# AtomGradient/swift-qwen3-tts

Measured on AMD Instinct MI355X. Metric: codec_tokens_per_s, higher is better.
Workload: dtype bf16

## Files before the change

### include/q3tts.h

```cpp
#ifndef Q3TTS_H
#define Q3TTS_H

#include <stddef.h>
#include <stdint.h>

#ifdef __cplusplus
extern "C" {
#endif

#define Q3TTS_ABI_VERSION 4

typedef struct q3tts_model q3tts_model;

typedef enum {
    Q3TTS_OK = 0,
    Q3TTS_ERR_MODEL_NOT_INITIALIZED = 1,
    Q3TTS_ERR_GENERATION_FAILED = 2,
    Q3TTS_ERR_INVALID_INPUT = 3,
    Q3TTS_ERR_AUDIO_DECODING_FAILED = 4,
    Q3TTS_ERR_AUDIO_ENCODING_FAILED = 5,
    Q3TTS_ERR_IO = 6,
    Q3TTS_ERR_DEVICE = 7,
    Q3TTS_ERR_CANCELLED = 8,
    Q3TTS_ERR_BUSY = 9
} q3tts_status;

typedef struct {
    int32_t device;
    int32_t max_batch;
    int32_t max_frames;
    int32_t max_prompt;
    int32_t use_graph;
    int32_t weights_from_broadcast;
    int32_t n_streams;
    int32_t codec_overlap_cus;
    int32_t codec_fp32;
    int32_t output_sample_rate;
    float speed;
    int32_t request_speeds;
} q3tts_load_opts;

void q3tts_default_load_opts(q3tts_load_opts* o);

typedef struct {
    q3tts_load_opts base;
    float pitch;
} q3tts_load_opts_ex;

void q3tts_default_load_opts_ex(q3tts_load_opts_ex* o);

q3tts_status q3tts_model_load(const char* model_dir, const q3tts_load_opts* opts, q3tts_model** out);
q3tts_status q3tts_model_load_ex(const char* model_dir, const q3tts_load_opts_ex* opts, q3tts_model** out);
void q3tts_model_free(q3tts_model* m);

const char* q3tts_last_error(const q3tts_model* m);

q3tts_status q3tts_model_arena(q3tts_model* m, void** device_ptr, size_t* bytes);

typedef struct {
    char tts_model_type[32];
    int32_t sample_rate;
    int32_t supports_voice_cloning;
    int32_t has_voice_cloning;
    int32_t hidden_size, num_layers, vocab_size, text_vocab_size, num_code_groups;
    int32_t cp_hidden_size, cp_num_layers, cp_vocab_size;
    int32_t codec_eos_token_id;
    int32_t samples_per_frame;
    int32_t max_batch;
    int64_t weight_bytes;
    int32_t speaker_embedding_dim;
    int32_t max_samples_per_frame;
} q3tts_model_info;
q3tts_status q3tts_model_get_info(const q3tts_model* m, q3tts_model_info* out);

typedef struct { char bytes[128]; } q3tts_comm_id;
q3tts_status q3tts_comm_get_unique_id(q3tts_comm_id* out);
q3tts_status q3tts_model_broadcast(q3tts_model* m, const q3tts_comm_id* id, int32_t rank, int32_t world, int32_t root);
q3tts_status q3tts_model_arena_checksum(q3tts_model* m, uint64_t* out);

int32_t q3tts_model_num_speakers(const q3tts_model* m);
const char* q3tts_model_speaker_name(const q3tts_model* m, int32_t i);

typedef struct {
    const int32_t* text_ids;
    int32_t n_text_ids;
    const int32_t* instruct_ids;
    int32_t n_instruct_ids;
    int32_t target_token_count;
    const char* speaker;
    const char* language;
    int32_t max_tokens;
    float speed;
    const float* ref_audio;
    int64_t n_ref_samples;
    const int32_t* ref_text_ids;
    int32_t n_ref_text_ids;
    int32_t route;
} q3tts_request;

#define Q3TTS_ROW_TEMPERATURE        1u
#define Q3TTS_ROW_TOP_K              2u
#define Q3TTS_ROW_TOP_P              4u
#define Q3TTS_ROW_REPETITION_PENALTY 8u
#define Q3TTS_ROW_SEED               16u
typedef struct {
    uint32_t set;
    float temperature;
    int32_t top_k;
    float top_p;
    float repetition_penalty;
    uint64_t seed;
} q3tts_row_sampling;

typedef struct {
    float temperature;
    int32_t top_k;
    float top_p;
    float repetition_penalty;
    uint64_t seed;
    int32_t force_frames;
    int32_t audio_chunk_frames;
    int32_t audio_window_frames;
    int32_t audio_lookahead_frames;
    uint32_t row_base;
    const q3tts_row_sampling* per_request;
    int32_t audio_stream_reference;
} q3tts_sampling;
void q3tts_default_sampling(q3tts_sampling* s);

typedef struct {
    int32_t prompt_token_count;
    int32_t generation_token_count;
    double prefill_time;
    double generate_time;
    double tokens_per_second;
    double peak_memory_usage;
} q3tts_gen_info;

typedef enum {
    Q3TTS_EVENT_TOKEN = 0, Q3TTS_EVENT_INFO = 1, Q3TTS_EVENT_AUDIO = 2,
    Q3TTS_EVENT_AUDIO_CHUNK = 3
} q3tts_event_kind;
typedef struct {
    q3tts_event_kind kind;
    int32_t request_index;
    int32_t token;
    const q3tts_gen_info* info;
    const float* pcm;
    int64_t n_samples;
    int64_t sample_offset;
} q3tts_event;
typedef void (*q3tts_event_cb)(void* user, const q3tts_event* ev);

typedef struct {
    q3tts_status status;
    float* pcm;
    int64_t n_samples;
    int32_t* codes;
    int32_t n_frames;
    q3tts_gen_info info;
} q3tts_result;

q3tts_status q3tts_generate(q3tts_model* m, const q3tts_request* reqs, int32_t n_reqs,
                            const q3tts_sampling* sampling, q3tts_event_cb cb, void* user,
                            q3tts_result* results);
void q3tts_result_free(q3tts_result* results, int32_t n);

typedef struct q3tts_job q3tts_job;
q3tts_status q3tts_generate_begin(q3tts_model* m, const q3tts_request* reqs, int32_t n_reqs,
                                  const q3tts_sampling* sampling, q3tts_event_cb cb, void* user, int32_t more_follows,
                                  q3tts_job** job);
q3tts_status q3tts_generate_end(q3tts_model* m, q3tts_job* job, q3tts_result* results);

q3tts_status q3tts_generate_queued(q3tts_model* m, const q3tts_request* reqs, int32_t n_reqs, int32_t slots,
                                   const q3tts_sampling* sampling, q3tts_event_cb cb, void* user, q3tts_result* results);

typedef struct q3tts_voice q3tts_voice;
q3tts_status q3tts_voice_create(q3tts_model* m, const float* ref_audio, int64_t n_ref_samples, const int32_t* ref_text_ids,
                                int32_t n_ref_text_ids, q3tts_voice** out);
q3tts_status q3tts_voice_create_rate(q3tts_model* m, const float* ref_audio, int64_t n_ref_samples, int32_t sample_rate,
                                     const int32_t* ref_text_ids, int32_t n_ref_text_ids, q3tts_voice** out);
void q3tts_voice_free(q3tts_model* m, q3tts_voice* v);
typedef struct {
    int32_t ref_frames, ref_text_tokens;
    int64_t n_ref_samples, device_bytes;
} q3tts_voice_info;
q3tts_status q3tts_voice_get_info(const q3tts_voice* v, q3tts_voice_info* out);
q3tts_status q3tts_generate_voices(q3tts_model* m, const q3tts_request* reqs, const q3tts_voice* const* voices, int32_t n_reqs,
                                   const q3tts_sampling* sampling, q3tts_event_cb cb, void* user, q3tts_result* results);
q3tts_status q3tts_generate_queued_voices(q3tts_model* m, const q3tts_request* reqs, const q3tts_voice* const* voices,
                                          int32_t n_reqs, int32_t slots, const q3tts_sampling* sampling, q3tts_event_cb cb,
                                          void* user, q3tts_result* results);

typedef struct q3tts_session q3tts_session;
typedef struct {
    int32_t slots;
    int32_t max_pending;
    int32_t max_ref_frames;
} q3tts_session_opts;
typedef struct {
    int64_t submitted, pending, running, completed, cancelled;
    int64_t frame_steps, admissions;
} q3tts_session_stats;
q3tts_status q3tts_session_open(q3tts_model* m, const q3tts_session_opts* opts, const q3tts_sampling* sampling, q3tts_event_cb cb,
                                void* user, q3tts_session** out);
q3tts_status q3tts_session_submit(q3tts_session* s, const q3tts_request* req, const q3tts_voice* voice ,
                                  const q3tts_row_sampling* rs , int64_t* ticket);
q3tts_status q3tts_session_cancel(q3tts_session* s, int64_t ticket);
q3tts_status q3tts_session_wait(q3tts_session* s, int64_t ticket, int32_t timeout_ms , q3tts_result* out,
                                int32_t* ready);
q3tts_status q3tts_session_get_stats(const q3tts_session* s, q3tts_session_stats* out);
q3tts_status q3tts_session_close(q3tts_session* s, int32_t drain);

typedef struct {
    int64_t open, starved, appended_tokens, starve_events;
} q3tts_session_text_stats;
q3tts_status q3tts_session_submit_open(q3tts_session* s, const q3tts_request* req, const q3tts_row_sampling* rs ,
                                       int64_t* ticket);
q3tts_status q3tts_session_append_text(q3tts_session* s, int64_t ticket, const int32_t* ids, int32_t n, int32_t final);
q3tts_status q3tts_session_get_text_stats(const q3tts_session* s, q3tts_session_text_stats* out);

q3tts_status q3tts_resample(q3tts_model* m, const float* in, int64_t n_in, int32_t in_rate, int32_t out_rate, int32_t centred,
                            float* out, int64_t cap, int64_t* n_out);

q3tts_status q3tts_model_get_speed(const q3tts_model* m, float* effective_speed, int32_t* hs, int32_t* delay_samples);
q3tts_status q3tts_time_stretch(q3tts_model* m, const float* in, int64_t n_in, float speed, int32_t causal, float* out, int64_t cap,
                                int64_t* n_out);

q3tts_status q3tts_model_get_pitch(const q3tts_model* m, float* effective_semitones, int32_t* hp, int32_t* ho, int32_t* delay_samples);
q3tts_status q3tts_pitch_shift(q3tts_model* m, const float* in, int64_t n_in, float semitones, float* out, int64_t cap, int64_t* n_out);

q3tts_status q3tts_request_speed_info(const q3tts_model* m, float speed, float* effective_speed, int32_t* hs, int32_t* delay_samples,
                                      int32_t* samples_per_frame);

q3tts_status q3tts_codec_decode(q3tts_model* m, const int32_t* codes, const int32_t* n_frames,
                                int32_t batch, int32_t max_frames, float* pcm, int64_t* audio_lengths);

q3tts_status q3tts_codec_decode_streamed(q3tts_model* m, const int32_t* codes, const int32_t* n_frames, int32_t batch,
                                         int32_t max_frames, int32_t chunk_frames, int32_t window, int32_t lookahead, float* pcm);

q3tts_status q3tts_codec_decode_streamed_prefixed(q3tts_model* m, const int32_t* codes, const int32_t* n_prefix, const int32_t* n_frames,
                                                  int32_t batch, int32_t max_frames, int32_t chunk_frames, int32_t window,
                                                  int32_t lookahead, float* pcm);

q3tts_status q3tts_codec_encode(q3tts_model* m, const float* audio, int64_t n_samples, int32_t* codes,
                                int32_t cap_frames, int32_t* n_frames);
int32_t q3tts_codec_encoded_frames(const q3tts_model* m, int64_t n_samples);

q3tts_status q3tts_speaker_embedding(q3tts_model* m, const float* audio, int64_t n_samples, int32_t sample_rate,
                                     float* out, int32_t cap);

void q3tts_pcm_to_int16(const float* pcm, int64_t n_samples, int16_t* out);
q3tts_status q3tts_write_wav(const char* path, const float* pcm, int64_t n_samples, int32_t sample_rate);

typedef struct q3tts_tokenizer q3tts_tokenizer;
q3tts_status q3tts_tokenizer_load(const char* path, q3tts_tokenizer** out);
void q3tts_tokenizer_free(q3tts_tokenizer* t);
q3tts_status q3tts_tokenizer_encode(const q3tts_tokenizer* t, const char* utf8, int32_t* ids, int32_t cap, int32_t* n);

typedef struct {
    double prefill_ms;
    double decode_ms;
    double codec_ms;
    int32_t frame_steps;
    int32_t rows;
    int64_t kv_bytes_read;
    double frontend_ms;
    double first_audio_ms;
    int32_t launches_per_frame_step;
} q3tts_timing;
q3tts_status q3tts_last_timing(const q3tts_model* m, q3tts_timing* out);


q3tts_status q3tts_debug_prepare_inputs(q3tts_model* m, const q3tts_request* req,
                                        uint16_t* input_embeds, int32_t cap_prompt, int32_t* n_prompt,
                                        uint16_t* trailing, int32_t cap_trailing, int32_t* n_trailing,
                                        uint16_t* tts_pad);

q3tts_status q3tts_debug_generate_forced(q3tts_model* m, const q3tts_request* reqs, int32_t n_reqs,
                                         const q3tts_sampling* sampling, const int32_t* forced_codes,
                                         int32_t n_frames, uint16_t* talker_logits, uint16_t* cp_logits,
                                         int32_t* sampled);

q3tts_status q3tts_debug_sample(q3tts_model* m, const uint16_t* logits, int32_t rows, int32_t V,
                                const q3tts_sampling* sampling, const uint8_t* seen,
                                int32_t suppress_lo, int32_t suppress_hi, int32_t eos_id,
                                uint32_t row0, uint32_t draw, int32_t* tokens);

q3tts_status q3tts_debug_text_resume(q3tts_model* m, int32_t H, int32_t V, const uint16_t* tables, const int32_t* codes,
                                     const uint16_t* text_row, uint16_t* out_h, float* out_ss, int32_t* out_state);

q3tts_status q3tts_debug_linear(q3tts_model* m, const uint16_t* x, const uint16_t* W, const uint16_t* bias,
                                int32_t M, int32_t K, int32_t N, uint16_t* y);

typedef struct {
    int32_t n_heads, n_kv, B;
    float eps, scale;
    int32_t max_pages;
    int32_t fixed_len;
    int32_t identity_pages;
    int32_t chunk;
    int32_t chunk_r_base;
    int32_t nt_kv;
    int32_t n_pos;
    int32_t n_pages;
    const uint16_t* qkv;
    const uint16_t* qn_w;
    const uint16_t* kn_w;
    const uint16_t* rope_cos;
    const uint16_t* rope_sin;
    const int32_t* kv_len;
    const uint8_t* active;
    const int32_t* block_table;
    const int32_t* chunk_n_prompt;
    uint16_t* kpool;
    uint16_t* vpool;
    uint16_t* out;
} q3tts_attn_debug;
q3tts_status q3tts_debug_attention(q3tts_model* m, const q3tts_attn_debug* a);

typedef struct {
    int32_t mode, geometry_only;
    int32_t M, K, N;
    int32_t xMB, yMB, ss_ld, y_cols;
    int32_t epi, act_silu, resid, nt_weights, y_tiled;
    int32_t norm, quant, has_bias;
    int32_t ss_count, norm_dim;
    float norm_eps;
    int32_t rider_M, rider_H, rider_MB, rider_ss_count;
    float rider_eps;
    int32_t rode;
    int32_t tall;
    int32_t tall_shape;
    int32_t split, mbw, nw, ch, np, gx, ntw;
    int32_t tm;
    const uint16_t* x;
    const void* W;
    const uint16_t* scales;
    const uint16_t* biases;
    const void* W_up;
    const uint16_t* scales_up;
    const uint16_t* biases_up;
    const uint16_t* bias;
    const uint16_t* norm_w;
    const float* ss_in;
    const uint16_t* rider_h;
    const uint16_t* rider_w;
    const float* rider_ss_in;
    uint16_t* y;
    float* ss_out;
    uint16_t* rider_out;
    float* rider_ss_out;
} q3tts_gemm_debug;
q3tts_status q3tts_debug_gemm(q3tts_model* m, q3tts_gemm_debug* a);

typedef struct {
    int32_t kind, geometry_only, split;
    int32_t B, Tmax, ppf, hist, margin;
    int32_t Cin, N, K, dil;
    int32_t ldx, ldo, ldr, ldx2;
    int32_t act, pre_act, shift, reflect, post_C;
    int32_t x_f32, res_is_out;
    int32_t family;
    int32_t BN;
    int32_t pro, pw_depth, KT, X32, CT2, PT, wdb;
    int32_t grid_x, grid_y, grid_z;
    int64_t lds_bytes;
    const int32_t* frames;
    const void* x;
    const float* x2;
    const float* w;
    const float* w2;
    const float* bias;
    const float* bias2;
    const float* scale;
    const float* snake_alpha;
    const float* snake_beta;
    const float* act2_alpha;
    const float* act2_beta;
    const float* post_alpha;
    const float* post_beta;
    const void* res;
    void* out;
    void* out2;
    float* pcm;
    int32_t* nonfinite;
} q3tts_conv_debug;
q3tts_status q3tts_debug_conv(q3tts_model* m, q3tts_conv_debug* a);

typedef struct {
    int32_t op, check_only;
    int32_t p[16];
    float f[4];
    const void* in[8];
    int64_t in_bytes[8];
    void* io[4];
    int64_t io_bytes[4];
} q3tts_rowop_debug;
q3tts_status q3tts_debug_rowop(q3tts_model* m, q3tts_rowop_debug* a);

typedef struct {
    float temperature;
    int32_t top_k;
    float top_p;
    float rep_penalty;
    uint64_t seed;
    uint32_t row0;
    int32_t mask_eos;
} q3tts_lm_sampling_params;
typedef struct {
    int32_t slot, n_trailing, max_frames;
    uint32_t row_key;
    int32_t text_open;
    int32_t pad_;
    q3tts_lm_sampling_params sp;
} q3tts_lm_admit_desc;
typedef struct {
    int32_t slot, src_row, n_new, close, max_frames, pad_;
} q3tts_lm_text_desc;
typedef struct {
    int32_t op, check_only;
    int32_t p[32];
    const void* in[14];
    int64_t in_bytes[14];
    void* io[18];
    int64_t io_bytes[18];
} q3tts_lmop_debug;
q3tts_status q3tts_debug_lmop(q3tts_model* m, q3tts_lmop_debug* a);

q3tts_status q3tts_debug_codec_stage(q3tts_model* m, const int32_t* codes, int32_t n_frames,
                                     const char* stage, float* out, int64_t cap_floats, int32_t* T, int32_t* C);

q3tts_status q3tts_debug_prefix_states(q3tts_model* m, int32_t* n_states, int64_t* device_bytes, int64_t* n_restored);

q3tts_status q3tts_debug_stretch_rows(q3tts_model* m, const float* x, const int32_t* lens, const int32_t* hops, int32_t B,
                                      int64_t x_stride, float* y, int64_t y_stride);

q3tts_status q3tts_debug_resample_ratio(q3tts_model* m, const float* x, const int32_t* lens, int32_t B, int64_t row_stride, int64_t in_units,
                                        int64_t out_units, int32_t centred, int32_t clamp, int32_t hist, float* y, int64_t y_stride);

q3tts_status q3tts_debug_codec_stream_slots(q3tts_model* m, const int32_t* codes, const int32_t* n_frames, int32_t n_reqs,
                                            int32_t max_frames, int32_t slots, int32_t burst, int32_t chunk_frames, int32_t window,
                                            int32_t lookahead, float* pcm);

q3tts_status q3tts_debug_build_decode_codes(q3tts_model* m, const int32_t* refs, const int32_t* ref_T, const int32_t* gen,
                                            const int32_t* n_frames, int32_t R, int32_t gen_stride, int32_t Fdec, int32_t misalign,
                                            int32_t* out);

void q3tts_debug_set_codec_scratch(uint64_t bytes);

void q3tts_debug_reload_env(void);

q3tts_status q3tts_debug_frontend_stage(q3tts_model* m, const float* audio, int64_t n_samples, const char* stage,
                                        float* out, int64_t cap_floats, int32_t* T, int32_t* C);

#ifdef __cplusplus
}
#endif
#endif
```

### swift-qwen3-tts_amd/csrc/debug_env.cc

```cpp
#include <atomic>
#include <cstdlib>
#include <mutex>

#include "kernels.h"

namespace q3 {

namespace {
std::mutex g_mu;
std::atomic<const DebugEnv*> g_env{nullptr};

bool flag(const char* name) { return std::getenv(name) != nullptr; }
int number(const char* name, int dflt) {
    const char* e = std::getenv(name);
    return e && *e ? std::atoi(e) : dflt;
}

const DebugEnv* read_env() {
    DebugEnv* d = new DebugEnv{};
    d->gemm_no_row_split = flag("Q3TTS_GEMM_NO_ROW_SPLIT");
    d->gemm_one_pair = flag("Q3TTS_GEMM_ONE_PAIR");
    d->gemm_parent_forms = number("Q3TTS_GEMM_PARENT_FORMS", 0) != 0;
    d->no_tall_gemm = flag("Q3TTS_NO_TALL_GEMM");
    d->tall_shape = number("Q3TTS_TALL_SHAPE", 0);
    d->chunk_qsplit = number("Q3TTS_CHUNK_QSPLIT", 0);
    d->conv_no_pw = flag("Q3TTS_CONV_NO_PW");
    d->nt_off = std::getenv("Q3TTS_NT") && number("Q3TTS_NT", 1) == 0;
    d->serial_jobs = number("Q3TTS_SERIAL_JOBS", 0) != 0;
    d->fail_back_half = number("Q3TTS_TEST_FAIL_BACK_HALF", 0) != 0;
    d->no_prefix_cache = number("Q3TTS_NO_PREFIX_CACHE", 0) != 0;
    return d;
}
}

const DebugEnv& debug_env() {
    const DebugEnv* e = g_env.load(std::memory_order_acquire);
    if (!e) {
        std::lock_guard<std::mutex> lk(g_mu);
        e = g_env.load(std::memory_order_acquire);
        if (!e) {
            e = read_env();
            g_env.store(e, std::memory_order_release);
        }
    }
    return *e;
}

void debug_env_reload() {
    std::lock_guard<std::mutex> lk(g_mu);
    g_env.store(read_env(), std::memory_order_release);
}

}
```

### swift-qwen3-tts_amd/csrc/engine_debug.cc

```cpp
#include "engine_stream.h"

#include "frontend.h"

namespace q3 {

void Engine::debug_frontend_stage(const float* audio, int64_t n_samples, const char* stage, float* out, int64_t cap, int* T, int* C) {
    Q3_CHECK(fe_ != nullptr, 1, "Model not initialized: Speech tokenizer encoder not available");
    Q3_CHECK(audio && n_samples > 0 && stage, 3, "Invalid input: empty audio or stage name");
    const float* a = upload_audio(audio, n_samples);
    StageCapture cap_s;
    cap_s.name = stage;
    static const char* kSpeaker[] = {"mel", "h0", "h1", "h2", "h3", "mfa", "pooled"};
    bool is_spk = false;
    for (const char* s : kSpeaker) is_spk = is_spk || cap_s.name == s;
    if (is_spk) {
        Q3_CHECK(m_->has_speaker_encoder, 1, "Model not initialized: Speaker encoder not available for this model");
        spk_f32_.grow(size_t(m_->cfg.talker.hidden_size));
        fe_->speaker_embedding(a, n_samples, spk_f32_, &cap_s);
    } else {
        Q3_CHECK(m_->has_codec_encoder, 1, "Model not initialized: Speech tokenizer encoder not available");
        const int Tq = fe_->encoded_frames(n_samples);
        ref_codes_dev_.grow(size_t(16) * Tq);
        fe_->encode(a, n_samples, ref_codes_dev_, &cap_s);
    }
    Q3_HIP(hipStreamSynchronize(st_));
    Q3_CHECK(!cap_s.data.empty(), 3, std::string("Invalid input: unknown front-end stage '") + stage + "'");
    Q3_CHECK(int64_t(cap_s.data.size()) <= cap, 3, "Invalid input: output buffer too small");
    std::memcpy(out, cap_s.data.data(), cap_s.data.size() * 4);
    *T = cap_s.T;
    *C = cap_s.C;
}

void Engine::debug_prepare_inputs(const q3tts_request& req, uint16_t* input_embeds, int cap_prompt, int* n_prompt,
                                  uint16_t* trailing, int cap_trailing, int* n_trailing, uint16_t* tts_pad) {
    q3tts_sampling sp{};
    q3tts_default_sampling(&sp);
    std::vector<ResolvedRequest> rr{resolve(req, sp)};
    if (rr[0].clone) prepare_clone_rows(rr);
    std::vector<int> np, nt;
    assemble_prompts(rr, np, nt);
    const int H = m_->cfg.talker.hidden_size;
    Q3_CHECK(np[0] <= cap_prompt && nt[0] <= cap_trailing, 3, "Invalid input: output buffers too small");
    Q3_HIP(hipStreamSynchronize(st_));
    Q3_HIP(hipMemcpy(input_embeds, prompt_, size_t(np[0]) * H * 2, hipMemcpyDeviceToHost));
    Q3_HIP(hipMemcpy(trailing, trailing_, size_t(nt[0]) * H * 2, hipMemcpyDeviceToHost));
    Q3_HIP(hipMemcpy(tts_pad, tts_pad_, size_t(H) * 2, hipMemcpyDeviceToHost));
    *n_prompt = np[0];
    *n_trailing = nt[0];
}

void Engine::debug_sample(const uint16_t* logits, int rows, int V, const q3tts_sampling& sp, const uint8_t* seen,
                          int suppress_lo, int suppress_hi, int eos_id, uint32_t row0, uint32_t draw, int32_t* tokens) {
    Q3_CHECK(rows >= 1 && rows <= Bm_ && V <= m_->cfg.talker.vocab_size, 3, "debug_sample: rows/V out of range");
    Q3_CHECK(draw % 16 == 0, 3, "debug_sample: draw must be a multiple of 16 (frame * 16)");
    const int Vt = m_->cfg.talker.vocab_size;
    Q3_HIP(hipMemcpy2D(tk_.logits, size_t(Vt) * 2, logits, size_t(V) * 2, size_t(V) * 2, size_t(rows), hipMemcpyHostToDevice));
    if (seen) Q3_HIP(hipMemcpy(seen_, seen, size_t(rows) * V, hipMemcpyHostToDevice));
    std::vector<int32_t> fr((size_t)(rows), int32_t(draw / 16)), big((size_t)(rows), 1 << 30);
    Q3_HIP(hipMemcpy(n_frames_, fr.data(), size_t(rows) * 4, hipMemcpyHostToDevice));
    Q3_HIP(hipMemcpy(max_frames_, big.data(), size_t(rows) * 4, hipMemcpyHostToDevice));
    Q3_HIP(hipMemset(finished_, 0, size_t(rows)));
    Q3_HIP(hipMemset(active_, 1, size_t(rows)));
    std::vector<SamplingParams> sph;
    for (int r = 0; r < rows; ++r) sph.push_back(fold_sampling(sp, r, row0));
    Q3_HIP(hipMemcpy(sp_dev_, sph.data(), sph.size() * sizeof(SamplingParams), hipMemcpyHostToDevice));
    SamplerArgs sa{};
    sa.logits = tk_.logits; sa.ldl = Vt; sa.V = V; sa.sp = sp_dev_;
    sa.is_talker = (eos_id >= 0 || suppress_hi > suppress_lo || seen) ? 1 : 0;
    sa.suppress_lo = suppress_lo; sa.suppress_hi = suppress_hi; sa.eos_id = eos_id;
    sa.seen = seen ? seen_ : nullptr; sa.cb = 0; sa.n_frames = n_frames_; sa.max_frames = max_frames_;
    sa.finished = finished_; sa.active = active_; sa.kv_len = kv_len_; sa.advance = 0;
    sa.cur_codes = cur_codes_; sa.codes = codes_; sa.Fmax = 0; sa.B = rows; sa.H = m_->cfg.talker.hidden_size;
    launch_sampler(sa, st_);
    Q3_HIP(hipStreamSynchronize(st_));
    std::vector<int32_t> cc((size_t)(rows) * 16);
    Q3_HIP(hipMemcpy(cc.data(), cur_codes_, cc.size() * 4, hipMemcpyDeviceToHost));
    for (int r = 0; r < rows; ++r) tokens[r] = cc[size_t(r) * 16];
    Q3_HIP(hipMemset(seen_, 0, size_t(rows) * V));
}

void Engine::debug_linear(const uint16_t* x, const uint16_t* W, const uint16_t* bias, int M, int K, int N, uint16_t* y) {
    Q3_CHECK(M >= 1 && M <= 1024 && K % 8 == 0 && N >= 1, 3, "debug_linear: unsupported shape");
    const int Kp = int(align_up(size_t(K), 128)), Np = int(align_up(size_t(N), 16)), Mp = int(align_up(size_t(M), 16));
    uint16_t *dW = nullptr, *dWt = nullptr, *dx = nullptr, *dy = nullptr, *db = nullptr;
    Q3_HIP(hipMalloc(reinterpret_cast<void**>(&dW), size_t(N) * K * 2));
    Q3_HIP(hipMalloc(reinterpret_cast<void**>(&dWt), size_t(Np) * Kp * 2));
    Q3_HIP(hipMalloc(reinterpret_cast<void**>(&dx), size_t(Mp) * Kp * 2));
    Q3_HIP(hipMalloc(reinterpret_cast<void**>(&dy), size_t(Mp) * Np * 2));
    Q3_HIP(hipMalloc(reinterpret_cast<void**>(&db), size_t(Np) * 2));
    Q3_HIP(hipMemset(dWt, 0, size_t(Np) * Kp * 2));
    Q3_HIP(hipMemset(dx, 0, size_t(Mp) * Kp * 2));
    Q3_HIP(hipMemset(db, 0, size_t(Np) * 2));
    Q3_HIP(hipMemcpy(dW, W, size_t(N) * K * 2, hipMemcpyHostToDevice));
    uint16_t* dxl = nullptr;
    Q3_HIP(hipMalloc(reinterpret_cast<void**>(&dxl), size_t(Mp) * Kp * 2));
    Q3_HIP(hipMemset(dxl, 0, size_t(Mp) * Kp * 2));
    Q3_HIP(hipMemcpy2D(dxl, size_t(Kp) * 2, x, size_t(K) * 2, size_t(K) * 2, size_t(M), hipMemcpyHostToDevice));
    launch_tile_rows(dxl, Kp, dx, Mp / 16, Mp, Kp, st_);
    if (bias) Q3_HIP(hipMemcpy(db, bias, size_t(N) * 2, hipMemcpyHostToDevice));
    launch_tile_weights(dW, N, K, dWt, Kp / 128, 0, 1, st_);
    LinearW L;
    L.w = dWt; L.bias = bias ? db : nullptr; L.N = N; L.K = K; L.Np = Np; L.Kp = Kp;
    GemmArgs ga{};
    ga.W = dWt; ga.x = dx; ga.xMB = Mp / 16; ga.M = M; ga.Mpad = Mp; ga.N = Np; ga.K = Kp; ga.epi = 0; ga.y = dy; ga.ldy = Np;
    ga.bias = L.bias; ga.ss_ld = Mp;
    launch_gemm_skinny(ga, st_);
    Q3_HIP(hipStreamSynchronize(st_));
    Q3_HIP(hipMemcpy2D(y, size_t(N) * 2, dy, size_t(Np) * 2, size_t(N) * 2, size_t(M), hipMemcpyDeviceToHost));
    for (void* p : {(void*)dW, (void*)dWt, (void*)dx, (void*)dxl, (void*)dy, (void*)db})
        if (p) (void)hipFree(p);
}

void Engine::debug_text_resume(int H, int V, const uint16_t* tables, const int32_t* codes, const uint16_t* text, uint16_t* out_h,
                               float* out_ss, int32_t* out_state) {
    Q3_CHECK(H >= 128 && H <= 4096 && H % 128 == 0 && V >= 1 && V <= 4096, 3, "debug_text_resume: H must be a multiple of 128 up to 4096, V up to 4096");
    Q3_CHECK(tables && codes && text && out_h && out_ss && out_state, 3, "Invalid input: null argument");
    for (int g = 0; g < 16; ++g) Q3_CHECK(codes[g] >= 0 && codes[g] < V, 3, "debug_text_resume: code outside the tables");
    constexpr int B = 2, row = 1, Tmax = 2;
    DevBuf<uint16_t> d_tab, d_trailing, d_pad, d_h, d_hl, d_text;
    DevBuf<const uint16_t*> d_cp;
    DevBuf<int32_t> d_i32;
    DevBuf<uint8_t> d_u8;
    DevBuf<float> d_ss;
    DevBuf<TextAppendDesc> d_desc;
    d_tab.grow(size_t(16) * V * H);
    d_trailing.grow(size_t(B) * Tmax * H);
    d_pad.grow(size_t(H));
    d_h.grow(size_t(16) * H);
    d_hl.grow(size_t(16) * H);
    d_text.grow(size_t(H));
    d_cp.grow(15);
    d_i32.grow(32 + 10);
    d_u8.grow(8);
    d_ss.grow(B);
    d_desc.grow(1);
    Q3_HIP(hipMemcpy(d_tab, tables, size_t(16) * V * H * 2, hipMemcpyHostToDevice));
    Q3_HIP(hipMemcpy(d_text, text, size_t(H) * 2, hipMemcpyHostToDevice));
    Q3_HIP(hipMemset(d_pad, 0, size_t(H) * 2));
    std::vector<const uint16_t*> cp(15);
    for (int g = 1; g < 16; ++g) cp[size_t(g - 1)] = d_tab + size_t(g) * V * H;
    Q3_HIP(hipMemcpy(d_cp, cp.data(), 15 * sizeof(const uint16_t*), hipMemcpyHostToDevice));
    int32_t* cur = d_i32;
    int32_t *n_tr = cur + 32, *t_idx = n_tr + 2, *n_fr = t_idx + 2, *max_fr = n_fr + 2, *cp_len = max_fr + 2;
    uint8_t *fin = d_u8, *act = fin + 2, *topen = act + 2, *starved = topen + 2;
    FrameEndArgs fe{};
    fe.cur_codes = cur; fe.codec_emb = d_tab; fe.cp_emb = d_cp;
    fe.trailing = d_trailing; fe.n_trailing = n_tr; fe.trailing_idx = t_idx; fe.Tmax = Tmax;
    fe.tts_pad = d_pad; fe.h = d_h; fe.hMB = 1; fe.ss_out = d_ss; fe.H = H; fe.B = B; fe.groups = 16;
    fe.n_frames = n_fr; fe.max_frames = max_fr; fe.finished = fin; fe.active = act; fe.cp_len = cp_len;
    fe.text_open = topen; fe.starved = starved;
    auto reset = [&](int n_trailing, int open) {
        std::vector<int32_t> hi(42, 0);
        for (int g = 0; g < 16; ++g) hi[size_t(16 + g)] = codes[g];
        hi[32 + row] = n_trailing;
        hi[38] = hi[39] = 100;
        hi[40] = hi[41] = 15;
        const uint8_t hu[8] = {1, 0, 0, 1, 0, uint8_t(open), 0, 0};
        const float hs[2] = {-1.f, -1.f};
        Q3_HIP(hipMemcpy(d_i32, hi.data(), hi.size() * 4, hipMemcpyHostToDevice));
        Q3_HIP(hipMemcpy(d_u8, hu, 8, hipMemcpyHostToDevice));
        Q3_HIP(hipMemcpy(d_ss, hs, 8, hipMemcpyHostToDevice));
        Q3_HIP(hipMemset(d_h, 0xEE, size_t(16) * H * 2));
        Q3_HIP(hipMemset(d_trailing, 0, size_t(B) * Tmax * H * 2));
    };
    auto read = [&](int k) {
        launch_untile_rows(d_h, 1, d_hl, H, 16, H, st_);
        Q3_HIP(hipStreamSynchronize(st_));
        Q3_HIP(hipMemcpy(out_h + size_t(k) * H, d_hl + size_t(row) * H, size_t(H) * 2, hipMemcpyDeviceToHost));
        float hs[2];
        int32_t hi[42];
        uint8_t hu[8];
        Q3_HIP(hipMemcpy(hs, d_ss, 8, hipMemcpyDeviceToHost));
        Q3_HIP(hipMemcpy(hi, d_i32, sizeof(hi), hipMemcpyDeviceToHost));
        Q3_HIP(hipMemcpy(hu, d_u8, 8, hipMemcpyDeviceToHost));
        out_ss[k] = hs[row];
        int32_t* o = out_state + size_t(k) * 8;
        o[0] = hi[36 + row]; o[1] = hi[34 + row]; o[2] = hi[32 + row]; o[3] = hu[row]; o[4] = hu[2 + row]; o[5] = hu[4 + row];
        o[6] = hu[6 + row]; o[7] = hi[40 + row];
    };
    reset(1, 0);
    Q3_HIP(hipMemcpy(d_trailing + size_t(row) * Tmax * H, d_text, size_t(H) * 2, hipMemcpyDeviceToDevice));
    launch_frame_end(fe, st_);
    read(0);
    reset(0, 1);
    launch_frame_end(fe, st_);
    read(1);
    TextAppendDesc d{};
    d.slot = row; d.src_row = 0; d.n_new = 1;
    Q3_HIP(hipMemcpy(d_desc, &d, sizeof(d), hipMemcpyHostToDevice));
    TextAppendArgs ta{};
    ta.desc = d_desc; ta.src = d_text; ta.eos_row = d_pad; ta.trailing = d_trailing; ta.n_trailing = n_tr; ta.text_open = topen;
    ta.max_frames = max_fr; ta.slots = B; ta.fe = fe;
    launch_text_append_rows(ta, &d, 1, st_);
    read(2);
}

void Engine::debug_build_decode_codes(const int32_t* refs, const int32_t* ref_T, const int32_t* gen, const int32_t* n_frames, int R,
                                      int gen_stride, int Fdec, bool misalign, int32_t* out) {
    size_t ref_total = 0;
    for (int r = 0; r < R; ++r) {
        Q3_CHECK(ref_T[r] >= 0 && n_frames[r] >= 0 && n_frames[r] <= gen_stride, 3, "Invalid input: frame counts out of range");
        ref_total += size_t(16) * ref_T[r];
    }
    Q3_CHECK(ref_total == 0 || refs, 3, "Invalid input: null argument");
    const size_t off = misalign ? 1 : 0, n_gen = size_t(R) * gen_stride * 16, n_out = size_t(R) * Fdec * 16;
    DevBuf<int32_t> d_ref, d_gen, d_out;
    DevBuf<DecodeRowDesc> d_desc;
    d_ref.grow(std::max<size_t>(ref_total, 1));
    d_gen.grow(n_gen + off);
    d_out.grow(n_out + off);
    d_desc.grow(size_t(R));
    if (ref_total) Q3_HIP(hipMemcpyAsync(d_ref, refs, ref_total * 4, hipMemcpyHostToDevice, st_));
    Q3_HIP(hipMemcpyAsync(d_gen + off, gen, n_gen * 4, hipMemcpyHostToDevice, st_));
    Q3_HIP(hipMemcpyAsync(d_out + off, out, n_out * 4, hipMemcpyHostToDevice, st_));
    std::vector<DecodeRowDesc> desc((size_t)(R));
    size_t at = 0;
    for (int r = 0; r < R; ++r) {
        desc[size_t(r)] = DecodeRowDesc{ref_T[r] > 0 ? d_ref + at : nullptr, d_gen + off + size_t(r) * gen_stride * 16, ref_T[r], n_frames[r], r, 0};
        at += size_t(16) * ref_T[r];
    }
    Q3_HIP(hipMemcpyAsync(d_desc, desc.data(), desc.size() * sizeof(DecodeRowDesc), hipMemcpyHostToDevice, st_));
    launch_build_decode_codes_rows(desc.data(), d_desc, R, d_out + off, R, Fdec, st_);
    Q3_HIP(hipMemcpyAsync(out, d_out + off, n_out * 4, hipMemcpyDeviceToHost, st_));
    Q3_HIP(hipStreamSynchronize(st_));
}

void Engine::debug_attention(const q3tts_attn_debug& d) {
    Q3_CHECK(d.qkv && d.qn_w && d.kn_w && d.rope_cos && d.rope_sin && d.kpool && d.vpool && d.out, 3, "debug_attention: null argument");
    Q3_CHECK(d.n_kv >= 1 && d.n_kv <= 64 && d.n_heads >= d.n_kv && d.n_heads % d.n_kv == 0 && d.n_heads / d.n_kv <= 4, 3,
             "debug_attention: unsupported GQA ratio");
    Q3_CHECK(d.B >= 1 && d.B <= 256, 3, "debug_attention: batch out of range");
    Q3_CHECK(d.chunk >= 0 && d.chunk <= 16, 3, "debug_attention: at most 16 positions per launch");
    Q3_CHECK(d.max_pages >= 1 && d.max_pages <= 64 && d.n_pages >= 1 && d.n_pages <= 4096 && d.n_pos >= 1 && d.n_pos <= 65536, 3,
             "debug_attention: sizes out of range");
    Q3_CHECK(d.fixed_len >= -1, 3, "debug_attention: fixed_len out of range");
    Q3_CHECK(d.fixed_len >= 0 || d.kv_len, 3, "debug_attention: kv_len missing");
    Q3_CHECK(d.identity_pages || d.block_table, 3, "debug_attention: block_table missing");
    Q3_CHECK(!d.identity_pages || d.B <= d.n_pages, 3, "debug_attention: identity_pages needs a page per row");
    const int B = d.B, C = std::max(d.chunk, 1), rows = C * B;
    const int cap = (d.identity_pages ? 1 : d.max_pages) * kPageTokens;
    for (int b = 0; b < B; ++b) {
        const int len0 = d.fixed_len >= 0 ? d.fixed_len : d.kv_len[b];
        int live = 1;
        if (d.chunk > 1 && d.chunk_n_prompt) {
            const int64_t r0 = int64_t(d.chunk_r_base) + d.chunk_n_prompt[b];
            live = r0 < 0 ? int(std::max<int64_t>(0, C + r0)) : C;
        } else if (d.chunk > 1) {
            live = C;
        }
        Q3_CHECK(len0 >= 0 && len0 <= cap && len0 + live <= cap && len0 + live <= d.n_pos, 3,
                 "debug_attention: cache length beyond the pages or the RoPE tables");
        if (!d.identity_pages)
            for (int pg = 0; pg * kPageTokens < len0 + live; ++pg) {
                const int32_t e = d.block_table[size_t(b) * d.max_pages + pg];
                Q3_CHECK(e >= 0 && e < d.n_pages, 3, "debug_attention: block-table entry outside the pool");
            }
    }
    const int ld = (d.n_heads + 2 * d.n_kv) * kHeadDim, odim = d.n_heads * kHeadDim;
    const int Mp = int(align_up(size_t(rows), 16));
    const size_t pool = size_t(d.n_pages) * d.n_kv * kPageTokens * kHeadDim;
    const size_t tab = size_t(d.n_pos) * kHeadDim;
    DevBuf<uint16_t> qkv, w, rope, kp, vp, ot, ol;
    DevBuf<int32_t> ints;
    DevBuf<uint8_t> act;
    qkv.grow(size_t(rows) * ld);
    w.grow(2 * kHeadDim);
    rope.grow(2 * tab);
    kp.grow(pool);
    vp.grow(pool);
    ot.grow(size_t(Mp) * odim);
    ol.grow(size_t(rows) * odim);
    ints.grow(size_t(B) * (2 + d.max_pages));
    act.grow(size_t(B));
    int32_t *kv_len = ints, *n_prompt = kv_len + B, *bt = n_prompt + B;
    Q3_HIP(hipMemset(ints, 0, size_t(B) * (2 + d.max_pages) * 4));
    Q3_HIP(hipMemcpy(qkv, d.qkv, size_t(rows) * ld * 2, hipMemcpyHostToDevice));
    Q3_HIP(hipMemcpy(w, d.qn_w, kHeadDim * 2, hipMemcpyHostToDevice));
    Q3_HIP(hipMemcpy(w + kHeadDim, d.kn_w, kHeadDim * 2, hipMemcpyHostToDevice));
    Q3_HIP(hipMemcpy(rope, d.rope_cos, tab * 2, hipMemcpyHostToDevice));
    Q3_HIP(hipMemcpy(rope + tab, d.rope_sin, tab * 2, hipMemcpyHostToDevice));
    Q3_HIP(hipMemcpy(kp, d.kpool, pool * 2, hipMemcpyHostToDevice));
    Q3_HIP(hipMemcpy(vp, d.vpool, pool * 2, hipMemcpyHostToDevice));
    if (d.kv_len) Q3_HIP(hipMemcpy(kv_len, d.kv_len, size_t(B) * 4, hipMemcpyHostToDevice));
    if (d.chunk_n_prompt) Q3_HIP(hipMemcpy(n_prompt, d.chunk_n_prompt, size_t(B) * 4, hipMemcpyHostToDevice));
    if (d.block_table) Q3_HIP(hipMemcpy(bt, d.block_table, size_t(B) * d.max_pages * 4, hipMemcpyHostToDevice));
    if (d.active) Q3_HIP(hipMemcpy(act, d.active, size_t(B), hipMemcpyHostToDevice));
    Q3_HIP(hipMemset(ot, 0xff, size_t(Mp) * odim * 2));
    AttnArgs at{};
    at.qkv = qkv; at.ld = ld; at.qn_w = w; at.kn_w = w + kHeadDim; at.eps = d.eps;
    at.rope_cos = rope; at.rope_sin = rope + tab;
    at.kpool = kp; at.vpool = vp;
    at.block_table = bt; at.max_pages = d.max_pages; at.kv_len = kv_len; at.active = d.active ? (const uint8_t*)act : nullptr;
    at.out = ot; at.outMB = Mp / 16; at.n_heads = d.n_heads; at.n_kv = d.n_kv; at.B = B;
    at.scale = d.scale;
    at.fixed_len = d.fixed_len; at.identity_pages = d.identity_pages ? 1 : 0;
    at.chunk = d.chunk; at.chunk_n_prompt = d.chunk_n_prompt ? n_prompt : nullptr; at.chunk_r_base = d.chunk_r_base;
    at.nt_kv = d.nt_kv ? 1 : 0;
    launch_attn_decode(at, st_);
    Q3_HIP(hipGetLastError());
    launch_untile_rows(ot, Mp / 16, ol, odim, rows, odim, st_);
    Q3_HIP(hipStreamSynchronize(st_));
    Q3_HIP(hipMemcpy(d.out, ol, size_t(rows) * odim * 2, hipMemcpyDeviceToHost));
    Q3_HIP(hipMemcpy(d.kpool, kp, pool * 2, hipMemcpyDeviceToHost));
    Q3_HIP(hipMemcpy(d.vpool, vp, pool * 2, hipMemcpyDeviceToHost));
}

void Engine::debug_gemm_check(q3tts_gemm_debug& d, GemmArgs& ga, NormRowsArgs& na) {
    static const uint16_t dummy16 = 0;
    static const uint32_t dummy32 = 0;
    d.rode = d.tall = d.tall_shape = d.split = d.mbw = d.nw = d.ch = d.np = d.gx = d.ntw = d.tm = 0;
    Q3_CHECK(d.mode == 0 || d.mode == 1, 3, "debug_gemm: unknown mode");
    const bool rider = d.mode == 1 || d.rider_M > 0;
    if (rider) {
        Q3_CHECK(d.rider_M >= 1 && d.rider_MB >= 1 && d.rider_MB <= 64 && d.rider_M <= 16 * d.rider_MB, 3, "debug_gemm: rider rows out of range");
        Q3_CHECK(d.rider_H >= 128 && d.rider_H <= 4096 && d.rider_H % 128 == 0, 3, "debug_gemm: rider_H must be a multiple of 128 up to 4096");
        Q3_CHECK(d.geometry_only || (d.rider_h && d.rider_w && d.rider_out), 3, "debug_gemm: null rider argument");
        if (d.rider_ss_in) Q3_CHECK(d.rider_ss_count >= 1 && d.rider_ss_count <= 256, 3, "debug_gemm: at most 256 partial sums of squares per rider row");
        na.hMB = na.outMB = d.rider_MB; na.eps = d.rider_eps; na.M = d.rider_M; na.H = d.rider_H;
        na.ss_count = d.rider_ss_in ? d.rider_ss_count : 0; na.ss_ld = 16 * d.rider_MB;
    }
    if (d.mode == 1) return;
    Q3_CHECK(d.epi == 0 || d.epi == 2 || d.epi == 3, 3, "debug_gemm: unknown epilogue");
    Q3_CHECK(d.M >= 1 && d.M <= 1024, 3, "debug_gemm: M out of range");
    Q3_CHECK(d.K >= 128 && d.K <= 8192 && d.K % 128 == 0, 3, "debug_gemm: K must be a multiple of 128 up to 8192");
    Q3_CHECK(d.N >= 8 && d.N <= 65536 && d.N % (d.epi == 2 ? 8 : 16) == 0, 3, "debug_gemm: N must be a multiple of 16 (epi 2: of 8)");
    const int Mp = int(align_up(size_t(d.M), 16));
    const bool tiled = d.epi != 0 || d.y_tiled;
    Q3_CHECK(d.xMB <= 64 && 16 * d.xMB >= Mp && d.yMB <= 64 && 16 * d.yMB >= Mp && d.ss_ld >= Mp && d.ss_ld <= 4096, 3,
             "debug_gemm: allocation smaller than the padded batch");
    Q3_CHECK(d.y_cols >= d.N && d.y_cols <= d.N + 1024 && d.y_cols % (tiled ? 128 : 8) == 0, 3, "debug_gemm: y_cols");
    Q3_CHECK(d.epi != 2 || (!d.has_bias && !d.act_silu), 3, "debug_gemm: the gate/up epilogue takes no bias or activation");
    Q3_CHECK(d.epi == 0 || !d.act_silu, 3, "debug_gemm: act_silu belongs to epi 0");
    Q3_CHECK(d.epi == 3 || (!d.resid && !d.ss_out), 3, "debug_gemm: resid / ss_out belong to epi 3");
    if (d.norm) Q3_CHECK(d.ss_count >= 1 && d.ss_count <= 4096 && d.norm_dim >= 1, 3, "debug_gemm: norm prologue sizes");
    if (!d.geometry_only) {
        Q3_CHECK(d.x && d.W && d.y, 3, "debug_gemm: null argument");
        Q3_CHECK((d.epi == 2) == (d.W_up != nullptr), 3, "debug_gemm: W_up goes with epi 2");
        Q3_CHECK((d.quant != 0) == (d.scales != nullptr) && (d.quant != 0) == (d.biases != nullptr), 3, "debug_gemm: scales / biases go with quant");
        if (d.epi == 2) Q3_CHECK((d.quant != 0) == (d.scales_up != nullptr) && (d.quant != 0) == (d.biases_up != nullptr), 3, "debug_gemm: scales / biases go with quant");
        Q3_CHECK((d.has_bias != 0) == (d.bias != nullptr), 3, "debug_gemm: bias goes with has_bias");
        Q3_CHECK((d.norm != 0) == (d.norm_w != nullptr) && (d.norm != 0) == (d.ss_in != nullptr), 3, "debug_gemm: norm_w / ss_in go with norm");
    }
    ga.Wsb = d.quant ? &dummy32 : nullptr;
    ga.xMB = d.xMB; ga.M = d.M; ga.Mpad = Mp; ga.N = d.N; ga.K = d.K; ga.epi = d.epi;
    ga.ldy = d.y_cols; ga.y_tiled = d.y_tiled ? 1 : 0; ga.yMB = d.yMB;
    ga.bias = d.has_bias ? &dummy16 : nullptr;
    ga.act_silu = d.act_silu ? 1 : 0;
    ga.norm_w = d.norm ? &dummy16 : nullptr;
    ga.ss_count = d.norm ? d.ss_count : 0; ga.ss_ld = d.ss_ld; ga.norm_dim = d.norm_dim; ga.norm_eps = d.norm_eps;
    ga.nt_weights = d.nt_weights ? 1 : 0; ga.resid = d.resid ? 1 : 0;
    const SkinnyGeom g = skinny_geometry(ga);
    d.tall = g.tall ? 1 : 0;
    if (g.tall) {
        d.tall_shape = gemm_tall_shape(ga);
    } else {
        Q3_CHECK(g.mbw >= 1 && g.mbw <= 4, 3, "debug_gemm: more than 4 row blocks per workgroup");
        d.split = g.split; d.mbw = g.mbw; d.nw = g.nw; d.ch = g.ch; d.np = g.np; d.gx = g.gx; d.ntw = g.ntw ? 1 : 0; d.tm = g.tm ? 1 : 0;
    }
    if (rider) d.rode = gemm_norm_rows_rides(ga, na) ? 1 : 0;
}

namespace {
void host_tile(const uint16_t* src, std::vector<uint16_t>& dst, int rows, int cols) {
    dst.resize(size_t(rows) * cols);
    for (int m = 0; m < rows; ++m)
        for (int k = 0; k < cols; k += 8) std::memcpy(&dst[act_tiled_offset(m, k, rows / 16)], src + size_t(m) * cols + k, 16);
}
void host_untile(const std::vector<uint16_t>& src, uint16_t* dst, int rows, int cols) {
    for (int m = 0; m < rows; ++m)
        for (int k = 0; k < cols; k += 8) std::memcpy(dst + size_t(m) * cols + k, &src[act_tiled_offset(m, k, rows / 16)], 16);
}
}

void Engine::debug_gemm(q3tts_gemm_debug& d) {
    GemmArgs ga{};
    NormRowsArgs na{};
    debug_gemm_check(d, ga, na);
    DevBuf<uint16_t> dx, dy, dbias, dnw, dsrc, dsc, dbi, rh, rw, rout;
    DevBuf<uint8_t> dWt;
    DevBuf<uint32_t> dWq, dsb;
    DevBuf<float> dssi, dsso, rssi, rsso;
    std::vector<uint16_t> tmp;
    auto up16 = [&](DevBuf<uint16_t>& b, const uint16_t* src, size_t n) {
        b.grow(n);
        Q3_HIP(hipMemcpy(b, src, n * 2, hipMemcpyHostToDevice));
    };
    const bool rider = d.mode == 1 || d.rider_M > 0;
    const int rrows = 16 * d.rider_MB;
    if (rider) {
        host_tile(d.rider_h, tmp, rrows, d.rider_H);
        up16(rh, tmp.data(), tmp.size());
        host_tile(d.rider_out, tmp, rrows, d.rider_H);
        up16(rout, tmp.data(), tmp.size());
        up16(rw, d.rider_w, size_t(d.rider_H));
        na.h = rh; na.w = rw; na.out = rout;
        if (d.rider_ss_in) {
            rssi.grow(size_t(d.rider_ss_count) * rrows);
            Q3_HIP(hipMemcpy(rssi, d.rider_ss_in, size_t(d.rider_ss_count) * rrows * 4, hipMemcpyHostToDevice));
            na.ss_in = rssi;
        }
        if (d.rider_ss_out) {
            rsso.grow(size_t(rrows));
            Q3_HIP(hipMemcpy(rsso, d.rider_ss_out, size_t(rrows) * 4, hipMemcpyHostToDevice));
            na.ss_out = rsso;
        }
    }
    const bool tiled = d.mode == 0 && (d.epi != 0 || d.y_tiled);
    const int yrows = 16 * d.yMB, n_tiles = d.mode == 0 ? (d.epi == 2 ? d.N / 8 : d.N / 16) : 0, KC = d.K / 128;
    const size_t n_ss_out = d.mode == 0 ? size_t(d.N / 16) * d.ss_ld : 0;
    if (d.mode == 0) {
        host_tile(d.x, tmp, 16 * d.xMB, d.K);
        up16(dx, tmp.data(), tmp.size());
        if (tiled) {
            host_tile(d.y, tmp, yrows, d.y_cols);
            up16(dy, tmp.data(), tmp.size());
        } else {
            up16(dy, d.y, size_t(yrows) * d.y_cols);
        }
        const size_t wbytes = d.quant ? size_t(n_tiles) * 16 * d.K / 2 : size_t(n_tiles) * 16 * d.K * 2;
        dWt.grow(wbytes);
        Q3_HIP(hipMemset(dWt, 0, wbytes));
        if (d.quant) {
            dsb.grow(size_t(n_tiles) * KC * 64);
            Q3_HIP(hipMemset(dsb, 0, size_t(n_tiles) * KC * 64 * 4));
        }
        const int rpt = d.epi == 2 ? 8 : 16;
        for (int part = 0; part < (d.epi == 2 ? 2 : 1); ++part) {
            const void* W = part ? d.W_up : d.W;
            if (d.quant) {
                dWq.grow(size_t(d.N) * d.K / 8);
                Q3_HIP(hipMemcpy(dWq, W, size_t(d.N) * d.K / 8 * 4, hipMemcpyHostToDevice));
                up16(dsc, part ? d.scales_up : d.scales, size_t(d.N) * d.K / 64);
                up16(dbi, part ? d.biases_up : d.biases, size_t(d.N) * d.K / 64);
                launch_tile_int4(dWq, dsc, dbi, d.N, d.K, dWt, dsb, KC, 0, 1, st_, rpt, 8 * part);
            } else {
                up16(dsrc, static_cast<const uint16_t*>(W), size_t(d.N) * d.K);
                launch_tile_weights(dsrc, d.N, d.K, reinterpret_cast<uint16_t*>(static_cast<uint8_t*>(dWt)), KC, 0, 1, st_, rpt, 8 * part);
            }
            Q3_HIP(hipStreamSynchronize(st_));
        }
        if (d.bias) up16(dbias, d.bias, size_t(d.N));
        if (d.norm) {
            up16(dnw, d.norm_w, size_t(d.K));
            dssi.grow(size_t(d.ss_count) * d.ss_ld);
            Q3_HIP(hipMemcpy(dssi, d.ss_in, size_t(d.ss_count) * d.ss_ld * 4, hipMemcpyHostToDevice));
        }
        if (d.ss_out) {
            dsso.grow(n_ss_out);
            Q3_HIP(hipMemcpy(dsso, d.ss_out, n_ss_out * 4, hipMemcpyHostToDevice));
        }
        ga.W = reinterpret_cast<const uint16_t*>(static_cast<uint8_t*>(dWt));
        ga.Wsb = d.quant ? static_cast<uint32_t*>(dsb) : nullptr;
        ga.x = dx; ga.y = dy;
        ga.bias = d.bias ? static_cast<uint16_t*>(dbias) : nullptr;
        ga.norm_w = d.norm ? static_cast<uint16_t*>(dnw) : nullptr;
        ga.ss_in = d.norm ? static_cast<float*>(dssi) : nullptr;
        ga.ss_out = d.ss_out ? static_cast<float*>(dsso) : nullptr;
    }
    bool launched = true;
    if (d.mode == 1) {
        launch_norm_rows(na, st_);
    } else if (rider) {
        launched = launch_gemm_skinny_with_norm_rows(ga, na, st_);
        Q3_CHECK(launched == (d.rode != 0), 7, "debug_gemm: the rider launch disagrees with gemm_norm_rows_rides");
    } else {
        launch_gemm_skinny(ga, st_);
    }
    Q3_HIP(hipGetLastError());
    Q3_HIP(hipStreamSynchronize(st_));
    if (!launched) return;
    if (d.mode == 0) {
        if (tiled) {
            tmp.resize(size_t(yrows) * d.y_cols);
            Q3_HIP(hipMemcpy(tmp.data(), dy, tmp.size() * 2, hipMemcpyDeviceToHost));
            host_untile(tmp, d.y, yrows, d.y_cols);
        } else {
            Q3_HIP(hipMemcpy(d.y, dy, size_t(yrows) * d.y_cols * 2, hipMemcpyDeviceToHost));
        }
        if (d.ss_out) Q3_HIP(hipMemcpy(d.ss_out, dsso, n_ss_out * 4, hipMemcpyDeviceToHost));
    }
    if (rider) {
        tmp.resize(size_t(rrows) * d.rider_H);
        Q3_HIP(hipMemcpy(tmp.data(), rout, tmp.size() * 2, hipMemcpyDeviceToHost));
        host_untile(tmp, d.rider_out, rrows, d.rider_H);
        if (d.rider_ss_out) Q3_HIP(hipMemcpy(d.rider_ss_out, rsso, size_t(rrows) * 4, hipMemcpyDeviceToHost));
    }
}

static void check_caller_codes(const CodecW& w, const int32_t* codes, const int32_t* n_frames, int batch, int max_frames) {
    for (int b = 0; b < batch; ++b)
        for (int f = 0; f < n_frames[b]; ++f) {
            const int32_t* c = codes + (size_t(b) * max_frames + f) * 16;
            Q3_CHECK(c[0] >= 0 && c[0] < w.cb_first_rows, 3, "Invalid input: first code outside the semantic codebook");
            for (size_t j = 0; j < w.cb_rest.size(); ++j)
                Q3_CHECK(c[1 + j] >= 0 && c[1 + j] < w.cb_rest_rows, 3, "Invalid input: code outside the acoustic codebook");
        }
}

void Engine::codec_decode(const int32_t* codes, const int32_t* n_frames, int batch, int max_frames, float* pcm,
                          int64_t* audio_lengths) {
    Q3_CHECK(m_->has_codec, 1, "Model not initialized: Speech tokenizer not loaded");
    Q3_CHECK(batch >= 1 && max_frames >= 1, 3, "Invalid input: empty codec batch");
    const int up = codec_->upsample();
    std::vector<int> frames((size_t)(batch));
    int Fmax = 0;
    for (int b = 0; b < batch; ++b) {
        Q3_CHECK(n_frames[b] >= 0 && n_frames[b] <= max_frames, 3, "Invalid input: n_frames out of range");
        frames[size_t(b)] = n_frames[b];
        Fmax = std::max(Fmax, n_frames[b]);
    }
    check_caller_codes(m_->codec, codes, n_frames, batch, max_frames);
    DevBuf<int32_t> dcodes;
    dcodes.grow(size_t(batch) * max_frames * 16);
    Q3_HIP(hipMemcpy(dcodes, codes, size_t(batch) * max_frames * 16 * 4, hipMemcpyHostToDevice));
    float* pcm_dev = nullptr;
    hipStream_t cst = codec_stream(false);
    PinnedBuf<int32_t> nf;
    nf.grow(size_t(batch));
    std::memset(nf, 0, size_t(batch) * 4);
    Q3_HIP(hipEventRecord(ev_[2], cst));
    if (Fmax > 0) codec_->decode(dcodes, max_frames, frames, &pcm_dev, std::string(), nullptr, nullptr, nullptr, nf);
    Q3_HIP(hipEventRecord(ev_[3], cst));
    Q3_HIP(hipStreamSynchronize(cst));
    bool bad = false;
    for (int b = 0; b < batch; ++b) bad = bad || nf[b] != 0;
    if (bad && !codec_->fp32_convs()) {
        std::memset(nf, 0, size_t(batch) * 4);
        codec_->decode(dcodes, max_frames, frames, &pcm_dev, std::string(), nullptr, nullptr, nullptr, nf, true);
        Q3_HIP(hipEventRecord(ev_[3], cst));
        Q3_HIP(hipStreamSynchronize(cst));
        bad = false;
        for (int b = 0; b < batch; ++b) bad = bad || nf[b] != 0;
    }
    if (bad) throw Error(4, kCodecRangeMsg);
    float ms = 0;
    Q3_HIP(hipEventElapsedTime(&ms, ev_[2], ev_[3]));
    timing.codec_ms = ms;
    for (int b = 0; b < batch; ++b) {
        const int F = frames[size_t(b)];
        if (F > 0)
            Q3_HIP(hipMemcpy(pcm + size_t(b) * max_frames * up, pcm_dev + size_t(b) * Fmax * up, size_t(F) * up * 4,
                             hipMemcpyDeviceToHost));
        int valid = 0;
        for (int f = 0; f < F; ++f) valid += codes[(size_t(b) * max_frames + f) * 16] > 0 ? 1 : 0;
        audio_lengths[b] = int64_t(valid) * up;
    }
}

void Engine::codec_decode_streamed(const int32_t* codes, const int32_t* n_frames, int batch, int max_frames, int chunk_frames, int window,
                                   int lookahead, float* pcm) {
    Q3_CHECK(m_->has_codec, 1, "Model not initialized: Speech tokenizer not loaded");
    Q3_CHECK(batch >= 1 && max_frames >= 1 && chunk_frames >= 1, 3, "Invalid input: empty codec batch");
    const int up = codec_->upsample();
    DevBuf<int32_t> dcodes;
    PinnedBuf<float> hpcm;
    struct Events {
        std::vector<hipEvent_t> v;
        ~Events() {
            for (auto e : v) (void)hipEventDestroy(e);
        }
    } done;
    dcodes.grow(size_t(batch) * max_frames * 16);
    Q3_HIP(hipMemcpy(dcodes, codes, size_t(batch) * max_frames * 16 * 4, hipMemcpyHostToDevice));
    hpcm.grow(size_t(batch) * max_frames * up);
    std::memset(hpcm, 0, size_t(batch) * max_frames * up * 4);
    std::vector<int> avail((size_t)(batch));
    std::vector<uint8_t> fin((size_t)(batch), 1);
    int Fmax = 0;
    for (int b = 0; b < batch; ++b) {
        Q3_CHECK(n_frames[b] >= 0 && n_frames[b] <= max_frames, 3, "Invalid input: n_frames out of range");
        avail[size_t(b)] = n_frames[b];
        Fmax = std::max(Fmax, n_frames[b]);
    }
    check_caller_codes(m_->codec, codes, n_frames, batch, max_frames);
    hipStream_t cst = codec_stream(false);
    CodecRunner::StreamCfg cfg;
    cfg.rows = batch; cfg.chunk_frames = chunk_frames; cfg.window = window; cfg.lookahead = lookahead; cfg.max_frames = std::max(Fmax, 1);
    codec_->stream_open(cfg);
    try {
        if (window >= 0) {
            std::vector<uint8_t> notyet((size_t)(batch), 0);
            for (int have = chunk_frames; have < Fmax + chunk_frames + lookahead; have += chunk_frames) {
                std::vector<int> a((size_t)(batch));
                for (int b = 0; b < batch; ++b) {
                    a[size_t(b)] = std::min(avail[size_t(b)], have);
                    notyet[size_t(b)] = a[size_t(b)] == avail[size_t(b)] ? 1 : 0;
                }
                codec_->stream_push(dcodes, max_frames, a.data(), notyet.data(), hpcm, size_t(max_frames) * up, done.v);
            }
        }
        codec_->stream_push(dcodes, max_frames, avail.data(), fin.data(), hpcm, size_t(max_frames) * up, done.v);
    } catch (...) {
        codec_->stream_close();
        throw;
    }
    codec_->stream_close();
    Q3_HIP(hipStreamSynchronize(cst));
    for (int b = 0; b < batch; ++b)
        std::memcpy(pcm + size_t(b) * max_frames * up, hpcm + size_t(b) * max_frames * up, size_t(n_frames[b]) * up * 4);
}

void Engine::codec_decode_streamed_prefixed(const int32_t* codes, const int32_t* n_prefix, const int32_t* n_frames, int batch, int max_frames,
                                            int chunk_frames, int window, int lookahead, float* pcm) {
    Q3_CHECK(m_->has_codec, 1, "Model not initialized: Speech tokenizer not loaded");
    Q3_CHECK(batch >= 1 && max_frames >= 1 && chunk_frames >= 1 && window >= 0 && lookahead >= 0, 3, "Invalid input: empty codec batch");
    Q3_CHECK(batch <= Bm_, 3, "Invalid input: batch must be between 1 and max_batch");
    int Fmax = 0, Rmax = 0;
    std::vector<int32_t> total((size_t)(batch));
    for (int b = 0; b < batch; ++b) {
        Q3_CHECK(n_prefix[b] >= 0 && n_frames[b] >= 0 && int64_t(n_prefix[b]) + n_frames[b] <= max_frames, 3,
                 "Invalid input: n_prefix + n_frames out of range");
        total[size_t(b)] = n_prefix[b] + n_frames[b];
        Fmax = std::max(Fmax, n_frames[b]);
        Rmax = std::max(Rmax, n_prefix[b]);
    }
    check_caller_codes(m_->codec, codes, total.data(), batch, max_frames);
    check_stream_chunk(chunk_frames);
    const int up = codec_->upsample();
    DevBuf<int32_t> dcodes;
    dcodes.grow(size_t(batch) * max_frames * 16);
    Q3_HIP(hipMemcpy(dcodes, codes, size_t(batch) * max_frames * 16 * 4, hipMemcpyHostToDevice));
    SlotStream ss(*this, batch, chunk_frames, window, lookahead, std::max(Fmax, 1), false, Rmax);
    ss.hold = false;
    for (int b = 0; b < batch; ++b) ss.admit(b, b, std::max(Fmax, 1), n_prefix[b]);
    std::vector<int> avail((size_t)(batch));
    std::vector<uint8_t> fin((size_t)(batch));
    for (int have = chunk_frames;; have += chunk_frames) {
        bool all = true;
        for (int b = 0; b < batch; ++b) {
            avail[size_t(b)] = std::min(n_frames[b], have);
            fin[size_t(b)] = avail[size_t(b)] == n_frames[b] ? 1 : 0;
            all = all && fin[size_t(b)];
        }
        ss.push(dcodes, max_frames, avail.data(), fin.data());
        if (all) break;
    }
    for (int b = 0; b < batch; ++b) ss.retire(b, n_frames[b]);
    ss.finish();
    for (int b = 0; b < batch; ++b) {
        Q3_CHECK(ss.out[b].complete, 7, "internal error: a row of the prefixed stream was left incomplete");
        std::memcpy(pcm + size_t(b) * Fmax * up, ss.out[b].pcm.get(), size_t(n_frames[b]) * up * 4);
    }
}

void Engine::debug_codec_stream_slots(const int32_t* codes, const int32_t* n_frames, int n_reqs, int max_frames, int slots, int burst,
                                      int chunk_frames, int window, int lookahead, float* pcm) {
    Q3_CHECK(m_->has_codec, 1, "Model not initialized: Speech tokenizer not loaded");
    Q3_CHECK(n_reqs >= 1 && max_frames >= 1 && burst >= 1 && chunk_frames >= 1 && window >= 0 && lookahead >= 0, 3,
             "Invalid input: empty codec batch");
    Q3_CHECK(slots >= 1 && slots <= Bm_, 3, "Invalid input: slots must be between 1 and max_batch");
    for (int i = 0; i < n_reqs; ++i) Q3_CHECK(n_frames[i] >= 0 && n_frames[i] <= max_frames, 3, "Invalid input: n_frames out of range");
    check_caller_codes(m_->codec, codes, n_frames, n_reqs, max_frames);
    check_stream_chunk(chunk_frames);
    const int up = codec_->upsample();
    DevBuf<int32_t> all, scodes;
    all.grow(size_t(n_reqs) * max_frames * 16);
    scodes.grow(size_t(slots) * max_frames * 16);
    Q3_HIP(hipMemcpy(all, codes, size_t(n_reqs) * max_frames * 16 * 4, hipMemcpyHostToDevice));
    SlotStream ss(*this, slots, chunk_frames, window, lookahead, max_frames, false);
    ss.hold = false;
    std::vector<int> copied((size_t)(slots), 0);
    replay_queue_schedule(
        n_frames, n_reqs, slots, burst,
        [&](int s, int r) {
            ss.admit(s, r, max_frames);
            copied[size_t(s)] = 0;
        },
        [&](const int* avail, const uint8_t* fin, const int* req) {
            for (int s = 0; s < slots; ++s) {
                if (req[s] < 0 || avail[s] <= copied[size_t(s)]) continue;
                Q3_HIP(hipMemcpyAsync(scodes + (size_t(s) * max_frames + copied[size_t(s)]) * 16,
                                      all + (size_t(req[s]) * max_frames + copied[size_t(s)]) * 16, size_t(avail[s] - copied[size_t(s)]) * 64,
                                      hipMemcpyDeviceToDevice, ss.cst));
                copied[size_t(s)] = avail[s];
            }
            ss.push(scodes, max_frames, avail, fin);
            for (int s = 0; s < slots; ++s)
                if (req[s] >= 0 && fin[s]) ss.retire(s, avail[s]);
        });
    ss.finish();
    for (int i = 0; i < n_reqs; ++i) {
        Q3_CHECK(ss.out[i].complete, 7, "internal error: a request of the slotted stream was left incomplete");
        std::memcpy(pcm + size_t(i) * max_frames * up, ss.out[i].pcm.get(), size_t(n_frames[i]) * up * 4);
    }
}

void Engine::debug_codec_stage(const int32_t* codes, int n_frames, const char* stage, float* out, int64_t cap, int* T, int* C) {
    Q3_CHECK(m_->has_codec, 1, "Model not initialized: Speech tokenizer not loaded");
    DevBuf<int32_t> dcodes;
    dcodes.grow(size_t(n_frames) * 16);
    Q3_HIP(hipMemcpy(dcodes, codes, size_t(n_frames) * 16 * 4, hipMemcpyHostToDevice));
    std::vector<float> so;
    float* pcm_dev = nullptr;
    (void)codec_stream(false);
    codec_->decode(dcodes, n_frames, {n_frames}, &pcm_dev, stage, &so, T, C);
    Q3_CHECK(int64_t(so.size()) <= cap, 3, "debug_codec_stage: output buffer too small");
    std::memcpy(out, so.data(), so.size() * 4);
}

}
```

### swift-qwen3-tts_amd/csrc/kernels.h

```cpp
#pragma once
#include <hip/hip_runtime.h>

#include <cstdint>

namespace q3 {

struct DebugEnv {
    bool gemm_no_row_split;
    bool gemm_one_pair;
    bool gemm_parent_forms;
    bool no_tall_gemm;
    int tall_shape;
    int chunk_qsplit;
    bool conv_no_pw;
    bool nt_off;
    bool serial_jobs;
    bool fail_back_half;
    bool no_prefix_cache;
};
const DebugEnv& debug_env();
void debug_env_reload();

constexpr int kPageTokens = 64;
constexpr int kHeadDim = 128;

struct NormRowsArgs {
    const uint16_t* h;
    int hMB;
    const uint16_t* w;
    float eps;
    uint16_t* out;
    int outMB;
    float* ss_out;
    int M, H;
    const float* ss_in;
    int ss_count, ss_ld;
};
void launch_norm_rows(const NormRowsArgs& a, hipStream_t st);

struct GemmArgs {
    const uint16_t* W;
    const uint32_t* Wsb;
    const uint16_t* x;
    int xMB;
    int M, Mpad, N, K;
    int epi;
    uint16_t* y;
    int ldy;
    int y_tiled, yMB;
    const uint16_t* bias;
    int act_silu;
    const uint16_t* norm_w;
    const float* ss_in;
    int ss_count, ss_ld, norm_dim;
    float norm_eps;
    int nt_weights;
    int resid;
    float* ss_out;
};
void launch_gemm_skinny(const GemmArgs& a, hipStream_t st);
struct SkinnyGeom {
    bool tall;
    int split, mbw;
    int nw, ch, np;
    int gx;
    bool ntw;
    bool tm;
};
SkinnyGeom skinny_geometry(const GemmArgs& a);
bool launch_gemm_skinny_with_norm_rows(const GemmArgs& a, const NormRowsArgs& n, hipStream_t st);
bool gemm_norm_rows_rides(const GemmArgs& a, const NormRowsArgs& n);
bool launch_gemm_tall(const GemmArgs& a, hipStream_t st);
bool gemm_tall_takes(const GemmArgs& a);
int gemm_tall_shape(const GemmArgs& a);


struct AttnArgs {
    const uint16_t* qkv;
    int ld;
    const uint16_t* qn_w;
    const uint16_t* kn_w;
    float eps;
    const uint16_t* rope_cos;
    const uint16_t* rope_sin;
    uint16_t* kpool;
    uint16_t* vpool;
    const int32_t* block_table;
    int max_pages;
    const int32_t* kv_len;
    const uint8_t* active;
    uint16_t* out;
    int outMB;
    int n_heads, n_kv, B;
    float scale;
    int fixed_len;
    int identity_pages;
    int chunk;
    const int32_t* chunk_n_prompt;
    int chunk_r_base;
    int nt_kv;
};
void launch_attn_decode(const AttnArgs& a, hipStream_t st);

struct FrameEndArgs {
    const int32_t* cur_codes;
    const uint16_t* codec_emb;
    const uint16_t* const* cp_emb;
    const uint16_t* trailing;
    const int32_t* n_trailing;
    int32_t* trailing_idx;
    int Tmax;
    const uint16_t* tts_pad;
    uint16_t* h;
    int hMB, H, B, groups;
    float* ss_out;
    int32_t* n_frames;
    const int32_t* max_frames;
    uint8_t* finished;
    uint8_t* active;
    int32_t* cp_len;
    const uint8_t* text_open;
    uint8_t* starved;
};
void launch_frame_end(const FrameEndArgs& a, hipStream_t st);

struct SamplingParams {
    float temperature;
    int top_k;
    float top_p;
    float rep_penalty;
    uint64_t seed;
    uint32_t row0;
    int mask_eos;
};

struct SamplerArgs {
    const uint16_t* logits;
    int ldl, V;
    const SamplingParams* sp;
    int is_talker;
    int suppress_lo, suppress_hi, eos_id;
    uint8_t* seen;
    int cb;
    const int32_t* n_frames;
    const int32_t* max_frames;
    uint8_t* finished;
    uint8_t* active;
    int32_t* kv_len;
    int advance;
    const uint8_t* advance_gate;
    int32_t* cur_codes;
    int32_t* codes;
    int Fmax;
    const int32_t* forced;
    int forced_frames;
    int32_t* sampled;
    const uint16_t* emb;
    int emb_ld;
    uint16_t* next_x;
    int next_MB;
    int next_row0;
    float* next_ss;
    const float* emb_ss;
    int nss, next_ss_ld;
    int H;
    int B;
    uint16_t* logits_dump;
    int dump_ld, dump_off;
    const uint32_t* row_key;
};
void launch_sampler(const SamplerArgs& a, hipStream_t st);
void launch_sampler_with_frame_end(const SamplerArgs& a, const FrameEndArgs& fe, hipStream_t st);
void launch_ss_to_table(const float* ss, int ss_ld, float* dst, int nss, int rows, hipStream_t st);

void launch_gather_rows(const uint16_t* table, int ld, const int32_t* ids, const int32_t* token_map,
                        int n, int dim, uint16_t* out, int ldo, int out_MB, hipStream_t st);
void launch_tile_rows(const uint16_t* src, int lds, uint16_t* dst, int dstMB, int rows, int dim, hipStream_t st);
void launch_untile_rows(const uint16_t* src, int srcMB, uint16_t* dst, int ldd, int rows, int dim, hipStream_t st);
void launch_add_rows(const uint16_t* a, int lda, const uint16_t* b, int ldb, int rows, int dim,
                     uint16_t* out, int ldo, hipStream_t st);

struct PrefillLoadArgs {
    const uint16_t* prompt;
    const int32_t* n_prompt;
    int Pmax, step, H, B;
    uint16_t* h;
    int hMB;
    float* ss_out;
    uint8_t* active;
};
void launch_prefill_load(const PrefillLoadArgs& a, hipStream_t st);
void launch_advance_len(int32_t* kv_len, const uint8_t* active, int B, hipStream_t st);
void launch_stamp(unsigned long long* acc, unsigned long long* last, int k, hipStream_t st);
void launch_prefill_chunk_load(const PrefillLoadArgs& a, int C, hipStream_t st);
void launch_advance_len_chunk(int32_t* kv_len, const int32_t* n_prompt, int r_base, int C, int B, hipStream_t st);

struct AdmitDesc {
    int32_t slot, n_trailing, max_frames;
    uint32_t row_key;
    int32_t text_open;
    SamplingParams sp;
};
struct AdmitArgs {
    const AdmitDesc* desc;
    const uint16_t* src_h;
    int srcMB;
    const float* src_ss;
    const int32_t* src_kv_len;
    const int32_t* src_n_prompt;
    uint16_t* h;
    int hMB;
    float* ss;
    int H, V, Fmax, slots;
    int32_t *kv_len, *n_prompt, *n_trailing, *max_frames, *n_frames, *cp_len, *trailing_idx, *cur_codes, *codes;
    uint32_t* row_key;
    SamplingParams* sp;
    uint8_t *finished, *active, *seen;
    uint8_t *text_open, *starved;
};
void launch_admit_rows(const AdmitArgs& a, int k, hipStream_t st);
void launch_cancel_rows(uint64_t mask, uint8_t* finished, uint8_t* active, int slots, hipStream_t st);
struct TextAppendDesc {
    int32_t slot, src_row, n_new, close, max_frames, pad_;
};
struct TextAppendArgs {
    const TextAppendDesc* desc;
    const uint16_t* src;
    const uint16_t* eos_row;
    uint16_t* trailing;
    int32_t* n_trailing;
    uint8_t* text_open;
    int32_t* max_frames;
    int slots;
    FrameEndArgs fe;
};
void launch_text_append_rows(const TextAppendArgs& a, const TextAppendDesc* host, int k, hipStream_t st);


void launch_compose_rows(const uint16_t* proj, int ldp, const uint16_t* table, int ldt, const uint16_t* extra, int lde,
                         const int32_t* a, const int32_t* b, const int32_t* dst_row, uint16_t* dst, int ldd, int n, int dim,
                         hipStream_t st);
void launch_ref_embed_rows(const int32_t* codes, int T, int groups, const uint16_t* codec_emb, const uint16_t* const* cp_emb,
                           int H, uint16_t* out, int ldo, hipStream_t st);
void launch_f32_to_bf16(const float* x, uint16_t* out, int n, hipStream_t st);
struct DecodeRowDesc {
    const int32_t* ref;
    const int32_t* gen;
    int32_t Tref, F, dst_row, pad_;
};
void launch_build_decode_codes_rows(const DecodeRowDesc* host, const DecodeRowDesc* rows, int R, int32_t* out, int out_rows,
                                    int Fdec, hipStream_t st);

void launch_copy_rows(const uint16_t* src, int lds, uint16_t* dst, int ldd, int rows, int dim, hipStream_t st);

}
```

### swift-qwen3-tts_amd/csrc/kernels/attn_body.inc

```
constexpr int D = kHeadDim;
constexpr int kMaxRep = 4;

__device__ __forceinline__ void norm_rope(float x0, float x1, const uint16_t* w, float eps, const uint16_t* cosr,
                                          const uint16_t* sinr, int lane, float& o0, float& o1) {
    float ss = wave_sum(x0 * x0 + x1 * x1);
    float rstd = 1.0f / sqrtf(ss / (float)D + eps);
    float y0 = rbf(rbf(x0 * rstd) * bf2f(w[lane]));
    float y1 = rbf(rbf(x1 * rstd) * bf2f(w[lane + 64]));
    o0 = rbf(rbf(y0 * bf2f(cosr[lane])) + rbf(-y1 * bf2f(sinr[lane])));
    o1 = rbf(rbf(y1 * bf2f(cosr[lane + 64])) + rbf(y0 * bf2f(sinr[lane + 64])));
}

template <int REP, int NTH, bool NTKV = false>
__device__ __forceinline__ void attn_decode_body(const AttnArgs& a, const int kvh, const int b) {
    constexpr int NG = NTH / 16;
    constexpr int NWV = NTH / 64;
    __shared__ __attribute__((aligned(16))) float q_s[REP][D];
    __shared__ float k_s[D];
    __shared__ float v_s[D];
    __shared__ float m_s[NG][REP];
    __shared__ float l_s[NG][REP];
    __shared__ float acc_s[NG][REP][D];

    const int tid = threadIdx.x, lane = tid & 63, wave = tid >> 6;
    const int len = a.fixed_len >= 0 ? a.fixed_len : a.kv_len[b];
    const bool append = a.active ? (a.active[b] != 0) : true;
    const uint16_t* row = a.qkv + (size_t)b * a.ld;
    const uint16_t* cosr = a.rope_cos + (size_t)len * D;
    const uint16_t* sinr = a.rope_sin + (size_t)len * D;
    const int qdim = a.n_heads * D, kdim = a.n_kv * D;

    const int32_t* bt = a.block_table + (size_t)b * a.max_pages;
    const int npage = a.identity_pages ? b : bt[len / kPageTokens];
    const size_t nslot = (((size_t)npage * a.n_kv + kvh) * kPageTokens + (len % kPageTokens)) * D;

    constexpr int VPW = (REP + 2 + NWV - 1) / NWV;
    uint16_t raw0[VPW], raw1[VPW];
#pragma unroll
    for (int u = 0; u < VPW; ++u) {
        const int j = wave + u * NWV;
        raw0[u] = 0;
        raw1[u] = 0;
        if (j < REP + 2) {
            const uint16_t* vp = row + (j < REP ? (size_t)(kvh * REP + j) * D : (j == REP ? qdim + (size_t)kvh * D : qdim + kdim + (size_t)kvh * D));
            raw0[u] = vp[lane];
            raw1[u] = vp[lane + 64];
        }
    }
    const uint16_t qw0 = a.qn_w[lane], qw1 = a.qn_w[lane + 64], kw0 = a.kn_w[lane], kw1 = a.kn_w[lane + 64];
    const uint16_t c0 = cosr[lane], c1 = cosr[lane + 64], s0 = sinr[lane], s1 = sinr[lane + 64];
    constexpr int PF = NTH >= 256 ? 8 : 4;
    const int g = tid >> 4, c = tid & 15;
    uint4 kpre[PF], vpre[PF];
#pragma unroll
    for (int u = 0; u < PF; ++u) {
        const int t = g + u * NG;
        kpre[u] = make_uint4(0, 0, 0, 0);
        vpre[u] = make_uint4(0, 0, 0, 0);
        if (t < len) {
            const int page = a.identity_pages ? b : bt[t / kPageTokens];
            const size_t off = (((size_t)page * a.n_kv + kvh) * kPageTokens + (t % kPageTokens)) * D + 8 * c;
            kpre[u] = ld16<NTKV>(reinterpret_cast<const uint4*>(a.kpool + off));
            vpre[u] = ld16<NTKV>(reinterpret_cast<const uint4*>(a.vpool + off));
        }
    }

    auto norm_rope_r = [&](float x0, float x1, uint16_t w0, uint16_t w1, float& o0, float& o1) {
        const float ss = wave_sum(x0 * x0 + x1 * x1);
        const float rstd = 1.0f / sqrtf(ss / (float)D + a.eps);
        const float y0 = rbf(rbf(x0 * rstd) * bf2f(w0));
        const float y1 = rbf(rbf(x1 * rstd) * bf2f(w1));
        o0 = rbf(rbf(y0 * bf2f(c0)) + rbf(-y1 * bf2f(s0)));
        o1 = rbf(rbf(y1 * bf2f(c1)) + rbf(y0 * bf2f(s1)));
    };
#pragma unroll
    for (int u = 0; u < VPW; ++u) {
        const int j = wave + u * NWV;
        if (j >= REP + 2) continue;
        if (j < REP) {
            float o0, o1;
            norm_rope_r(bf2f(raw0[u]), bf2f(raw1[u]), qw0, qw1, o0, o1);
            q_s[j][lane] = o0;
            q_s[j][lane + 64] = o1;
        } else if (j == REP) {
            float o0, o1;
            norm_rope_r(bf2f(raw0[u]), bf2f(raw1[u]), kw0, kw1, o0, o1);
            k_s[lane] = o0;
            k_s[lane + 64] = o1;
            if (append) {
                a.kpool[nslot + lane] = f2bf(o0);
                a.kpool[nslot + lane + 64] = f2bf(o1);
            }
        } else {
            v_s[lane] = bf2f(raw0[u]);
            v_s[lane + 64] = bf2f(raw1[u]);
            if (append) {
                a.vpool[nslot + lane] = raw0[u];
                a.vpool[nslot + lane + 64] = raw1[u];
            }
        }
    }
    __syncthreads();

    float q[REP][8];
#pragma unroll
    for (int h = 0; h < REP; ++h)
#pragma unroll
        for (int j = 0; j < 8; ++j) q[h][j] = q_s[h][8 * c + j];
    float m[REP], l[REP], acc[REP][8];
#pragma unroll
    for (int h = 0; h < REP; ++h) {
        m[h] = -INFINITY;
        l[h] = 0.f;
#pragma unroll
        for (int j = 0; j < 8; ++j) acc[h][j] = 0.f;
    }

    auto step = [&](const float (&kf)[8], const float (&vf)[8]) {
#pragma unroll
        for (int h = 0; h < REP; ++h) {
            float d = 0.f;
#pragma unroll
            for (int j = 0; j < 8; ++j) d += q[h][j] * kf[j];
            d = row16_sum(d);
            const float sc = d * a.scale;
            const float mn = fmaxf(m[h], sc);
            const float alpha = __expf(m[h] - mn);
            const float p = __expf(sc - mn);
            l[h] = l[h] * alpha + p;
#pragma unroll
            for (int j = 0; j < 8; ++j) acc[h][j] = acc[h][j] * alpha + p * vf[j];
            m[h] = mn;
        }
    };

    auto step_raw = [&](const uint4& kr, const uint4& vr) {
        float kf[8] = {lo_bf(kr.x), hi_bf(kr.x), lo_bf(kr.y), hi_bf(kr.y), lo_bf(kr.z), hi_bf(kr.z), lo_bf(kr.w), hi_bf(kr.w)};
        float vf[8] = {lo_bf(vr.x), hi_bf(vr.x), lo_bf(vr.y), hi_bf(vr.y), lo_bf(vr.z), hi_bf(vr.z), lo_bf(vr.w), hi_bf(vr.w)};
        step(kf, vf);
    };
#pragma unroll
    for (int u = 0; u < PF; ++u)
        if (g + u * NG < len) step_raw(kpre[u], vpre[u]);
    for (int t0 = g + PF * NG; t0 < len; t0 += PF * NG) {
        uint4 kr[PF], vr[PF];
#pragma unroll
        for (int u = 0; u < PF; ++u) {
            const int t = t0 + u * NG;
            kr[u] = make_uint4(0, 0, 0, 0);
            vr[u] = make_uint4(0, 0, 0, 0);
            if (t < len) {
                const int page = a.identity_pages ? b : bt[t / kPageTokens];
                const size_t off = (((size_t)page * a.n_kv + kvh) * kPageTokens + (t % kPageTokens)) * D + 8 * c;
                kr[u] = ld16<NTKV>(reinterpret_cast<const uint4*>(a.kpool + off));
                vr[u] = ld16<NTKV>(reinterpret_cast<const uint4*>(a.vpool + off));
            }
        }
#pragma unroll
        for (int u = 0; u < PF; ++u)
            if (t0 + u * NG < len) step_raw(kr[u], vr[u]);
    }
    if (g == (len % NG)) {
        float kf[8], vf[8];
#pragma unroll
        for (int j = 0; j < 8; ++j) {
            kf[j] = k_s[8 * c + j];
            vf[j] = v_s[8 * c + j];
        }
        step(kf, vf);
    }

#pragma unroll
    for (int h = 0; h < REP; ++h) {
        if (c == 0) {
            m_s[g][h] = m[h];
            l_s[g][h] = l[h];
        }
#pragma unroll
        for (int j = 0; j < 8; ++j) acc_s[g][h][8 * c + j] = acc[h][j];
    }
    __syncthreads();

    uint16_t* out_s = reinterpret_cast<uint16_t*>(&q_s[0][0]);
    for (int o = tid; o < REP * D; o += NTH) {
        const int h = o / D, d = o % D;
        float M = -INFINITY;
#pragma unroll
        for (int gg = 0; gg < NG; ++gg) M = fmaxf(M, m_s[gg][h]);
        float num = 0.f, den = 0.f;
#pragma unroll
        for (int gg = 0; gg < NG; ++gg) {
            const float w = (m_s[gg][h] == -INFINITY) ? 0.f : __expf(m_s[gg][h] - M);
            num += acc_s[gg][h][d] * w;
            den += l_s[gg][h] * w;
        }
        out_s[o] = f2bf(num / den);
    }
    __syncthreads();
    for (int p = tid; p < REP * D / 8; p += NTH) {
        const int col = (kvh * REP) * D + 8 * p;
        *reinterpret_cast<uint4*>(a.out + act_tiled_offset(b, col, a.outMB)) = *reinterpret_cast<const uint4*>(out_s + 8 * p);
    }
}
```

### swift-qwen3-tts_amd/csrc/kernels/attn_decode.hip

```cpp
#include <algorithm>
#include <cstdlib>

#include <type_traits>

#include "../common.h"
#include "../kernels.h"

namespace q3 {
namespace {

#include "attn_body.inc"

template <int REP, int NTH, bool NTKV = false>
__global__ __launch_bounds__(NTH) void attn_decode_kernel(AttnArgs a) {
    __builtin_amdgcn_s_setprio(3);
    attn_decode_body<REP, NTH, NTKV>(a, blockIdx.x, blockIdx.y);
}

template <int REP, int NTH, int CMAX>
__global__ __launch_bounds__(NTH) void attn_chunk_kernel(AttnArgs a) {
    __builtin_amdgcn_s_setprio(3);
    constexpr int NG = NTH / 16;
    constexpr int NWV = NTH / 64;
    __shared__ __attribute__((aligned(16))) float q_s[CMAX][REP][D];
    using KV = typename std::conditional<(CMAX > 8), uint16_t, float>::type;
    auto kv_put = [](float v) -> KV { if constexpr (CMAX > 8) return f2bf(v); else return v; };
    auto kv_get = [](KV v) -> float { if constexpr (CMAX > 8) return bf2f(v); else return v; };
    __shared__ KV k_s[CMAX][D];
    __shared__ KV v_s[CMAX][D];
    __shared__ float m_s[NG][REP];
    __shared__ float l_s[NG][REP];
    __shared__ float acc_s[NG][REP][D];
    __shared__ __attribute__((aligned(16))) uint16_t out_s[REP * D];

    const int kvh = blockIdx.x, b = blockIdx.y;
    const int tid = threadIdx.x, lane = tid & 63, wave = tid >> 6;
    const int C = a.chunk;
    const int len0 = a.fixed_len >= 0 ? a.fixed_len : a.kv_len[b];
    const int r0 = a.chunk_n_prompt ? a.chunk_r_base + a.chunk_n_prompt[b] : 0;
    const int p0 = r0 < 0 ? (-r0 < C ? -r0 : C) : 0;
    const int qdim = a.n_heads * D, kdim = a.n_kv * D;
    const int32_t* bt = a.block_table + (size_t)b * a.max_pages;

    const int qs = blockIdx.z, nqs = gridDim.z;
    for (int vtx = wave; vtx < (C - p0) * (REP + 2); vtx += NWV) {
        const int p = p0 + vtx / (REP + 2), j = vtx % (REP + 2);
        if (j < REP && p % nqs != qs) continue;
        const int pos = len0 + (p - p0);
        const uint16_t* row = a.qkv + (size_t)(p * a.B + b) * a.ld;
        const uint16_t* cosr = a.rope_cos + (size_t)pos * D;
        const uint16_t* sinr = a.rope_sin + (size_t)pos * D;
        const int npage = a.identity_pages ? b : bt[pos / kPageTokens];
        const size_t nslot = (((size_t)npage * a.n_kv + kvh) * kPageTokens + (pos % kPageTokens)) * D;
        if (j < REP) {
            const uint16_t* qp = row + (size_t)(kvh * REP + j) * D;
            float o0, o1;
            norm_rope(bf2f(qp[lane]), bf2f(qp[lane + 64]), a.qn_w, a.eps, cosr, sinr, lane, o0, o1);
            q_s[p][j][lane] = o0;
            q_s[p][j][lane + 64] = o1;
        } else if (j == REP) {
            const uint16_t* kp = row + qdim + (size_t)kvh * D;
            float o0, o1;
            norm_rope(bf2f(kp[lane]), bf2f(kp[lane + 64]), a.kn_w, a.eps, cosr, sinr, lane, o0, o1);
            k_s[p][lane] = kv_put(o0);
            k_s[p][lane + 64] = kv_put(o1);
            if (qs == 0) {
                a.kpool[nslot + lane] = f2bf(o0);
                a.kpool[nslot + lane + 64] = f2bf(o1);
            }
        } else {
            const uint16_t* vp = row + qdim + kdim + (size_t)kvh * D;
            const uint16_t v0 = vp[lane], v1 = vp[lane + 64];
            v_s[p][lane] = kv_put(bf2f(v0));
            v_s[p][lane + 64] = kv_put(bf2f(v1));
            if (qs == 0) {
                a.vpool[nslot + lane] = v0;
                a.vpool[nslot + lane + 64] = v1;
            }
        }
    }
    __syncthreads();

    const int g = tid >> 4, c = tid & 15;
    for (int p = p0; p < C; ++p) {
        if (p % nqs != qs) continue;
        float q[REP][8];
#pragma unroll
        for (int h = 0; h < REP; ++h)
#pragma unroll
            for (int j = 0; j < 8; ++j) q[h][j] = q_s[p][h][8 * c + j];
        float m[REP], l[REP], acc[REP][8];
#pragma unroll
        for (int h = 0; h < REP; ++h) {
            m[h] = -INFINITY;
            l[h] = 0.f;
#pragma unroll
            for (int j = 0; j < 8; ++j) acc[h][j] = 0.f;
        }
        auto step = [&](const float (&kf)[8], const float (&vf)[8]) {
#pragma unroll
            for (int h = 0; h < REP; ++h) {
                float d = 0.f;
#pragma unroll
                for (int j = 0; j < 8; ++j) d += q[h][j] * kf[j];
                d = row16_sum(d);
                const float sc = d * a.scale;
                const float mn = fmaxf(m[h], sc);
                const float alpha = __expf(m[h] - mn);
                const float pr = __expf(sc - mn);
                l[h] = l[h] * alpha + pr;
#pragma unroll
                for (int j = 0; j < 8; ++j) acc[h][j] = acc[h][j] * alpha + pr * vf[j];
                m[h] = mn;
            }
        };
        const int len = len0 + (p - p0);
        for (int t = g; t <= len; t += NG) {
            float kf[8], vf[8];
            if (t < len0) {
                const int page = a.identity_pages ? b : bt[t / kPageTokens];
                const size_t off = (((size_t)page * a.n_kv + kvh) * kPageTokens + (t % kPageTokens)) * D + 8 * c;
                const uint4 kr = *reinterpret_cast<const uint4*>(a.kpool + off);
                const uint4 vr = *reinterpret_cast<const uint4*>(a.vpool + off);
                kf[0] = lo_bf(kr.x); kf[1] = hi_bf(kr.x); kf[2] = lo_bf(kr.y); kf[3] = hi_bf(kr.y);
                kf[4] = lo_bf(kr.z); kf[5] = hi_bf(kr.z); kf[6] = lo_bf(kr.w); kf[7] = hi_bf(kr.w);
                vf[0] = lo_bf(vr.x); vf[1] = hi_bf(vr.x); vf[2] = lo_bf(vr.y); vf[3] = hi_bf(vr.y);
                vf[4] = lo_bf(vr.z); vf[5] = hi_bf(vr.z); vf[6] = lo_bf(vr.w); vf[7] = hi_bf(vr.w);
            } else {
                const int e = p0 + (t - len0);
#pragma unroll
                for (int j = 0; j < 8; ++j) {
                    kf[j] = kv_get(k_s[e][8 * c + j]);
                    vf[j] = kv_get(v_s[e][8 * c + j]);
                }
            }
            step(kf, vf);
        }
#pragma unroll
        for (int h = 0; h < REP; ++h) {
            if (c == 0) {
                m_s[g][h] = m[h];
                l_s[g][h] = l[h];
            }
#pragma unroll
            for (int j = 0; j < 8; ++j) acc_s[g][h][8 * c + j] = acc[h][j];
        }
        __syncthreads();
        for (int o = tid; o < REP * D; o += NTH) {
            const int h = o / D, d = o % D;
            float M = -INFINITY;
#pragma unroll
            for (int gg = 0; gg < NG; ++gg) M = fmaxf(M, m_s[gg][h]);
            float num = 0.f, den = 0.f;
#pragma unroll
            for (int gg = 0; gg < NG; ++gg) {
                const float w = (m_s[gg][h] == -INFINITY) ? 0.f : __expf(m_s[gg][h] - M);
                num += acc_s[gg][h][d] * w;
                den += l_s[gg][h] * w;
            }
            out_s[o] = f2bf(num / den);
        }
        __syncthreads();
        for (int pc = tid; pc < REP * D / 8; pc += NTH) {
            const int col = (kvh * REP) * D + 8 * pc;
            *reinterpret_cast<uint4*>(a.out + act_tiled_offset(p * a.B + b, col, a.outMB)) = *reinterpret_cast<const uint4*>(out_s + 8 * pc);
        }
        __syncthreads();
    }
}

}

void launch_attn_decode(const AttnArgs& a, hipStream_t st) {
    const int rep = a.n_heads / a.n_kv;
    Q3_CHECK(rep * a.n_kv == a.n_heads && rep >= 1 && rep <= kMaxRep, 3, "attn_decode: unsupported GQA ratio");
    dim3 grid(a.n_kv, a.B);
    const bool wide = a.max_pages > 1 && rep <= 2;
    if (a.chunk > 1) {
        Q3_CHECK(a.chunk <= 16, 3, "attn_decode: at most 16 positions per launch");
        const int qenv = debug_env().chunk_qsplit;
        const int nqs = qenv > 0 ? std::max(1, std::min(a.chunk, qenv)) : (a.chunk > 8 ? 2 : 1);
        const dim3 cgrid(a.n_kv, a.B, nqs);
#define Q3_CHUNK(REPv, NTHv)                                                                                        \
    do {                                                                                                            \
        if (a.chunk > 8) hipLaunchKernelGGL((attn_chunk_kernel<REPv, NTHv, 16>), cgrid, dim3(NTHv), 0, st, a);       \
        else hipLaunchKernelGGL((attn_chunk_kernel<REPv, NTHv, 8>), cgrid, dim3(NTHv), 0, st, a);                    \
    } while (0)
        switch (rep) {
            case 1: if (wide) Q3_CHUNK(1, 512); else Q3_CHUNK(1, 256); break;
            case 2: if (wide) Q3_CHUNK(2, 512); else Q3_CHUNK(2, 256); break;
            case 3: Q3_CHUNK(3, 256); break;
            case 4: Q3_CHUNK(4, 256); break;
        }
#undef Q3_CHUNK
        return;
    }
    switch (rep) {
        case 1:
            if (wide) hipLaunchKernelGGL((attn_decode_kernel<1, 512>), grid, dim3(512), 0, st, a);
            else hipLaunchKernelGGL((attn_decode_kernel<1, 256>), grid, dim3(256), 0, st, a);
            break;
        case 2:
            if (wide && a.nt_kv) hipLaunchKernelGGL((attn_decode_kernel<2, 512, true>), grid, dim3(512), 0, st, a);
            else if (wide) hipLaunchKernelGGL((attn_decode_kernel<2, 512>), grid, dim3(512), 0, st, a);
            else hipLaunchKernelGGL((attn_decode_kernel<2, 256>), grid, dim3(256), 0, st, a);
            break;
        case 3: hipLaunchKernelGGL((attn_decode_kernel<3, 256>), grid, dim3(256), 0, st, a); break;
        case 4: hipLaunchKernelGGL((attn_decode_kernel<4, 256>), grid, dim3(256), 0, st, a); break;
    }
}

}
```

### swift-qwen3-tts_amd/csrc/kernels/gemm_body.inc

```
#ifdef Q3TTS_GEMM_TIMELINE
__device__ unsigned long long g_gemm_tl[4][2][8][8];
#define Q3_TL_BEGIN()                                                                                                       \
    constexpr int kTlForm = (EPI == 2 && MB == 2 && NW == 8 && CH == 2 && NP == 3 && NTW) ? (TM ? 1 : 0)                    \
                            : ((EPI == 3 && MB == 1 && NW == 8 && CH == 6 && !NORM && NTW) ? 2                              \
                               : ((EPI == 0 && MB == 2 && NW == 8 && CH == 2 && NORM && NP == 1 && NTW) ? 3 : -1));         \
    unsigned long long tl_[8] = {0, 0, 0, 0, 0, 0, 0, 0};                                                                   \
    Q3_TL(0)
#define Q3_TL(k)                                   \
    do {                                           \
        if constexpr (kTlForm >= 0) {              \
            __builtin_amdgcn_sched_barrier(0);     \
            tl_[k] = wall_clock64();               \
            __builtin_amdgcn_sched_barrier(0);     \
        }                                          \
    } while (0)
#define Q3_TL_END()                                                                                                         \
    do {                                                                                                                    \
        if constexpr (kTlForm >= 0) {                                                                                       \
            const bool tl_last = blockIdx.x == gridDim.x - 1 && blockIdx.y == gridDim.y - 1;                                \
            if ((tl_last || (blockIdx.x == 0 && blockIdx.y == 0)) && lane == 0) {                                           \
                _Pragma("unroll") for (int k = 0; k < 8; ++k) g_gemm_tl[kTlForm][tl_last ? 1 : 0][wave][k] = tl_[k];        \
            }                                                                                                               \
        }                                                                                                                   \
    } while (0)
#else
#define Q3_TL_BEGIN() ((void)0)
#define Q3_TL(k) ((void)0)
#define Q3_TL_END() ((void)0)
#endif

__device__ __forceinline__ f32x4 mfma16(const uint4& a, const uint4& b, f32x4 c) {
    bf16x8 av, bv;
    __builtin_memcpy(&av, &a, 16);
    __builtin_memcpy(&bv, &b, 16);
    return __builtin_amdgcn_mfma_f32_16x16x32_bf16(av, bv, c, 0, 0, 0);
}

__device__ __forceinline__ float silu_f(float v) { return v / (1.0f + __expf(-v)); }

__device__ __forceinline__ uint4 norm8(const uint4& hx, const uint4& wx, float rstd) {
    const uint32_t hw[4] = {hx.x, hx.y, hx.z, hx.w}, ww[4] = {wx.x, wx.y, wx.z, wx.w};
    uint32_t o[4];
#pragma unroll
    for (int j = 0; j < 4; ++j) {
        const float n0 = rbf(lo_bf(hw[j]) * rstd), n1 = rbf(hi_bf(hw[j]) * rstd);
        o[j] = pack_bf(n0 * lo_bf(ww[j]), n1 * hi_bf(ww[j]));
    }
    return make_uint4(o[0], o[1], o[2], o[3]);
}

__device__ __forceinline__ void dequant_chunk(const uint4& qw, uint32_t sb, uint4 (&out)[4]) {
    const float sc = lo_bf(sb), bi = hi_bf(sb);
    const uint32_t w[4] = {qw.x, qw.y, qw.z, qw.w};
#pragma unroll
    for (int i = 0; i < 4; ++i) {
        uint32_t o[4];
#pragma unroll
        for (int j = 0; j < 4; ++j) {
            const float q0 = (float)((w[i] >> (8 * j)) & 15u), q1 = (float)((w[i] >> (8 * j + 4)) & 15u);
            o[j] = pack_bf(__fadd_rn(__fmul_rn(q0, sc), bi), __fadd_rn(__fmul_rn(q1, sc), bi));
        }
        out[i] = make_uint4(o[0], o[1], o[2], o[3]);
    }
}

template <int MB, int EPI, int NW, int CH, bool NORM, bool QUANT, int NP = 1, bool NTW = false, bool TM = false>
__device__ __forceinline__ void gemm_skinny_body(const GemmArgs& a, const int tile, const int mb0) {
    constexpr int NT = NP;
    constexpr int NR = 1;
    constexpr int NB = TM ? NT : 1;
    constexpr int kDefer = TM ? NT - 1 : 0;
    static_assert(!TM || (EPI == 2 && NORM && !QUANT && CH > 0 && NP > 1), "tile-major order is a gate/up form");
    const int n_tiles = (EPI == 2) ? (a.N >> 3) : (a.N >> 4);
    __shared__ float red[NB][NW][NR][MB][4][64];
    __shared__ __attribute__((aligned(16))) uint16_t ys[NB][MB][16][16];
    __shared__ float rstd_s[NORM ? 16 * MB : 1];
    __shared__ float ssp_s[NORM ? 8 : 1][NORM ? 16 * MB : 1];

    const int lane = threadIdx.x & 63;
    const int wave = threadIdx.x >> 6;
    Q3_TL_BEGIN();
    const int KC = a.K >> 7;

    f32x4 acc[NT][MB];
#pragma unroll
    for (int t = 0; t < NT; ++t)
#pragma unroll
        for (int mb = 0; mb < MB; ++mb) acc[t][mb] = f32x4{0.f, 0.f, 0.f, 0.f};

    const uint4* Wt = reinterpret_cast<const uint4*>(a.W);
    const uint4* Xt = reinterpret_cast<const uint4*>(a.x);

    constexpr int kSsIter = NORM ? (16 * MB * 8 + NW * 64 - 1) / (NW * 64) : 1;
    float sst[kSsIter][16];
    if constexpr (NORM) {
        const int rows = 16 * MB;
#pragma unroll
        for (int it = 0; it < kSsIter; ++it) {
            const int idx = (threadIdx.x + it * NW * 64) % (rows * 8);
            const int row = idx % rows, part = idx / rows;
            const float* sp = a.ss_in + 16 * mb0 + row;
#pragma unroll
            for (int u = 0; u < 16; ++u) {
                const int j = part + 8 * u;
                sst[it][u] = sp[(size_t)(j < a.ss_count ? j : 0) * a.ss_ld];
            }
        }
        __builtin_amdgcn_sched_barrier(0);
    }

    constexpr int CHR = CH > 0 ? CH : 1;
    constexpr int WL = QUANT ? 1 : 4;
    uint4 wf[CHR][NT][WL];
    uint32_t wsb[CHR][NT];
    auto load_w = [&](int c, int kc, int t0, int t1) {
#pragma unroll
        for (int t = t0; t < t1; ++t) {
            const int tt = tile * NT + t;
            const size_t blk = (size_t)(tt < n_tiles ? tt : n_tiles - 1) * KC + kc;
            if constexpr (QUANT) {
                wf[c][t][0] = ld16<NTW>(Wt + blk * 64 + lane);
                wsb[c][t] = a.Wsb[blk * 64 + lane];
            } else {
                const uint4* wp = Wt + blk * 256 + lane;
#pragma unroll
                for (int i = 0; i < 4; ++i) wf[c][t][i] = ld16<NTW>(wp + i * 64);
            }
        }
    };

    constexpr int kWRegs = CH * NT * (QUANT ? 5 : 16);
    constexpr int kRoom = (((MB == 1 && !NORM) ? 200 : 176) - kWRegs) / (MB * 16);
    constexpr int kCap = (MB == 1 && !NORM) ? 6 : 3;
    constexpr int XG0 = (CH == 0) ? 0 : (kRoom < 1 ? 1 : (kRoom > kCap ? (CH < kCap ? CH : kCap) : (kRoom < CH ? kRoom : CH)));
    constexpr int XG = (MB == 2 && NORM && CH == 2 && NT == 1 && EPI == 0) ? 1 : XG0;
    static_assert(!TM || XG == CH, "tile-major order keeps every chunk's x fragments in registers");
    uint4 xr[XG > 0 ? XG : 1][MB][4];
    uint4 nwr[(NORM && XG > 0) ? XG : 1][4];
#pragma unroll
    for (int ph = 0; ph < 2; ++ph) {
        if (ph == 1) __builtin_amdgcn_sched_barrier(0);
        if ((ph == 0) != NORM) {
    if constexpr (TM) {
#pragma unroll
            for (int t = 0; t < NT - kDefer; ++t)
#pragma unroll
                for (int c = 0; c < CH; ++c) {
                    const int kl = wave + c * NW;
                    load_w(c, kl < KC ? kl : 0, t, t + 1);
                }
    } else if constexpr (CH > 0) {
#pragma unroll
            for (int c = 0; c < CH; ++c) {
                const int kl = wave + c * NW;
                load_w(c, kl < KC ? kl : 0, 0, NT);
            }
        }
        } else {
    if constexpr (XG > 0) {
#pragma unroll
        for (int c = 0; c < XG; ++c) {
            const int kl = wave + c * NW;
            const int kc = kl < KC ? kl : 0;
            if constexpr (NORM) {
                const uint4* np = reinterpret_cast<const uint4*>(a.norm_w + kc * 128 + 32 * (lane >> 4));
#pragma unroll
                for (int i = 0; i < 4; ++i) nwr[c][i] = np[i];
            }
#pragma unroll
            for (int mb = 0; mb < MB; ++mb) {
                const uint4* xp = Xt + ((size_t)(kc * a.xMB + mb0 + mb) * 4) * 64 + lane;
#pragma unroll
                for (int i = 0; i < 4; ++i) xr[c][mb][i] = xp[i * 64];
            }
        }
    }
        }
    }
    __builtin_amdgcn_sched_barrier(0);
    uint4 hv_pre = make_uint4(0, 0, 0, 0);
    if constexpr (EPI == 3 && NT == 1) {
        if (a.resid && threadIdx.x < 32 * MB) {
            const int o = threadIdx.x, mb = o >> 5, b = (o >> 1) & 15, p = o & 1;
            hv_pre = *reinterpret_cast<const uint4*>(a.y + act_tiled_offset(16 * (mb0 + mb) + b, tile * 16 + 8 * p, a.yMB));
        }
    }

    float rstd[MB];
    if constexpr (NORM) {
        const int rows = 16 * MB;
#pragma unroll
        for (int it = 0; it < kSsIter; ++it) {
            const int idx = threadIdx.x + it * NW * 64;
            if (idx < rows * 8) {
                const int row = idx % rows, part = idx / rows;
                float s = 0.f;
#pragma unroll
                for (int u = 0; u < 16; ++u)
                    if (part + 8 * u < a.ss_count) s += sst[it][u];
                for (int j = part + 128; j < a.ss_count; j += 8) s += a.ss_in[(size_t)j * a.ss_ld + 16 * mb0 + row];
                ssp_s[part][row] = s;
            }
        }
        __syncthreads();
        if (threadIdx.x < rows) {
            float s = 0.f;
#pragma unroll
            for (int p = 0; p < 8; ++p) s += ssp_s[p][threadIdx.x];
            rstd_s[threadIdx.x] = 1.0f / sqrtf(s / (float)a.norm_dim + a.norm_eps);
        }
        __syncthreads();
#pragma unroll
        for (int mb = 0; mb < MB; ++mb) rstd[mb] = rstd_s[16 * mb + (lane & 15)];
    }
    Q3_TL(1);
    if constexpr (TM) {
#pragma unroll
        for (int c = 0; c < CH; ++c) {
#pragma unroll
            for (int mb = 0; mb < MB; ++mb)
#pragma unroll
                for (int i = 0; i < 4; ++i) xr[c][mb][i] = norm8(xr[c][mb][i], nwr[c][i], rstd[mb]);
        }
        __builtin_amdgcn_sched_barrier(0);
#pragma unroll
        for (int t = NT - kDefer; t < NT; ++t)
#pragma unroll
            for (int c = 0; c < CH; ++c) {
                const int kl = wave + c * NW;
                load_w(c, kl < KC ? kl : 0, t, t + 1);
            }
        __builtin_amdgcn_sched_barrier(0);
    }

    auto chunk = [&](int kc, int c, const uint4 (*xpre)[4], const uint4* nwpre) {
        uint4 w[NT][4];
#pragma unroll
        for (int t = 0; t < NT; ++t) {
            if constexpr (QUANT) {
                dequant_chunk(wf[c][t][0], wsb[c][t], w[t]);
            } else {
#pragma unroll
                for (int i = 0; i < 4; ++i) w[t][i] = wf[c][t][i];
            }
        }
        uint4 nw[4];
        if constexpr (NORM) {
            if (nwpre) {
#pragma unroll
                for (int i = 0; i < 4; ++i) nw[i] = nwpre[i];
            } else {
                const uint4* np = reinterpret_cast<const uint4*>(a.norm_w + kc * 128 + 32 * (lane >> 4));
#pragma unroll
                for (int i = 0; i < 4; ++i) nw[i] = np[i];
            }
        }
#pragma unroll
        for (int mb = 0; mb < MB; ++mb) {
            uint4 xf[4];
            if (xpre) {
#pragma unroll
                for (int i = 0; i < 4; ++i) xf[i] = xpre[mb][i];
            } else {
                const uint4* xp = Xt + ((size_t)(kc * a.xMB + mb0 + mb) * 4) * 64 + lane;
#pragma unroll
                for (int i = 0; i < 4; ++i) xf[i] = xp[i * 64];
            }
            if constexpr (NORM) {
#pragma unroll
                for (int i = 0; i < 4; ++i) xf[i] = norm8(xf[i], nw[i], rstd[mb]);
            }
#pragma unroll
            for (int t = 0; t < NT; ++t)
#pragma unroll
                for (int i = 0; i < 4; ++i) acc[t][mb] = mfma16(w[t][i], xf[i], acc[t][mb]);
        }
    };
    if constexpr (TM) {
    } else if constexpr (CH > 0) {
#pragma unroll
        for (int g0 = 0; g0 < CH; g0 += XG) {
            if (g0 > 0) {
#pragma unroll
                for (int c = 0; c < XG; ++c) {
                    if (g0 + c < CH) {
                        const int kl = wave + (g0 + c) * NW;
                        const int kc = kl < KC ? kl : 0;
                        if constexpr (NORM) {
                            const uint4* np = reinterpret_cast<const uint4*>(a.norm_w + kc * 128 + 32 * (lane >> 4));
#pragma unroll
                            for (int i = 0; i < 4; ++i) nwr[c][i] = np[i];
                        }
#pragma unroll
                        for (int mb = 0; mb < MB; ++mb) {
                            const uint4* xp = Xt + ((size_t)(kc * a.xMB + mb0 + mb) * 4) * 64 + lane;
#pragma unroll
                            for (int i = 0; i < 4; ++i) xr[c][mb][i] = xp[i * 64];
                        }
                    }
                }
            }
#pragma unroll
            for (int c = 0; c < XG; ++c) {
                if (g0 + c < CH) {
                    const int kl = wave + (g0 + c) * NW;
                    if (kl < KC) chunk(kl, g0 + c, xr[c], NORM ? nwr[c] : nullptr);
                }
                if (g0 + c == 0) Q3_TL(2);
            }
        }
    } else {
        for (int kl = wave; kl < KC; kl += NW) {
            load_w(0, kl, 0, NT);
            chunk(kl, 0, nullptr, nullptr);
        }
    }

    if constexpr (!TM) Q3_TL(3);
#pragma unroll
    for (int pr = 0; pr < NT / NR; ++pr) {
    const int rb = TM ? pr : 0;
    if constexpr (TM) {
#pragma unroll
        for (int c = 0; c < CH; ++c) {
            if (wave + c * NW < KC) {
#pragma unroll
                for (int mb = 0; mb < MB; ++mb)
#pragma unroll
                    for (int i = 0; i < 4; ++i) acc[pr][mb] = mfma16(wf[c][pr][i], xr[c][mb][i], acc[pr][mb]);
            }
        }
        if (pr == 0) Q3_TL(2);
        if (pr == NT - 1) Q3_TL(3);
    } else {
        if (pr > 0) __syncthreads();
    }
#pragma unroll
    for (int t = 0; t < NR; ++t)
#pragma unroll
        for (int mb = 0; mb < MB; ++mb)
#pragma unroll
            for (int q = 0; q < 4; ++q) red[rb][wave][t][mb][q][lane] = acc[pr * NR + t][mb][q];
    __syncthreads();
    if (pr == NT / NR - 1) Q3_TL(4);
    const int otile = tile * (NT / NR) + pr;

    if constexpr (EPI == 2) {
        for (int o = threadIdx.x; o < 128 * MB; o += NW * 64) {
            const int mb = o >> 7, rem = o & 127;
            const int b = rem >> 3, f = rem & 7;
            const int lg = (f >> 2) * 16 + b, lu = (2 + (f >> 2)) * 16 + b, q = f & 3;
            float g = 0.f, u = 0.f;
#pragma unroll
            for (int w = 0; w < NW; ++w) {
                g += red[rb][w][0][mb][q][lg];
                u += red[rb][w][0][mb][q][lu];
            }
            ys[rb][mb][b][f] = f2bf(rbf(silu_f(rbf(g))) * rbf(u));
        }
    } else {
    for (int o = threadIdx.x; o < 256 * MB; o += NW * 64) {
        const int mb = o >> 8, rem = o & 255;
        const int b = rem >> 4, f = rem & 15;
        const int src_lane = (f >> 2) * 16 + b, q = f & 3;
        float sum = 0.f;
#pragma unroll
        for (int w = 0; w < NW; ++w) sum += red[rb][w][0][mb][q][src_lane];
        const int n = otile * 16 + f;
        float y = sum;
        if (a.bias && otile < n_tiles) y += bf2f(a.bias[n]);
        uint16_t yb = f2bf(y);
        if (EPI == 0 && a.act_silu) yb = f2bf(silu_f(bf2f(yb)));
        ys[rb][mb][b][f] = yb;
    }
    }
    __syncthreads();
    if (pr == 0) Q3_TL(7);
    if (pr == NT / NR - 1) Q3_TL(5);
    if constexpr (EPI == 2) {
        for (int o = threadIdx.x; o < 16 * MB; o += NW * 64) {
            const int mb = o >> 4, b = o & 15;
            const int m = 16 * (mb0 + mb) + b;
            if (m < a.M && otile < n_tiles)
                *reinterpret_cast<uint4*>(a.y + act_tiled_offset(m, otile * 8, a.yMB)) = *reinterpret_cast<const uint4*>(&ys[rb][mb][b][0]);
        }
    } else
    for (int o = threadIdx.x; o < 32 * MB; o += NW * 64) {
        const int mb = o >> 5, b = (o >> 1) & 15, p = o & 1;
        const int m = 16 * (mb0 + mb) + b;
        uint4 v = *reinterpret_cast<const uint4*>(&ys[rb][mb][b][8 * p]);
        const int n = otile * 16 + 8 * p;
        if constexpr (EPI == 3) {
            uint16_t* hp = a.y + act_tiled_offset(m, n, a.yMB);
            float ss = 0.f;
            const uint32_t yw[4] = {v.x, v.y, v.z, v.w};
            uint32_t ow[4];
            uint4 hv = hv_pre;
            if constexpr (NT > 1) {
                if (a.resid && m < a.M && otile < n_tiles) hv = *reinterpret_cast<const uint4*>(hp);
            }
            const uint32_t hw[4] = {hv.x, hv.y, hv.z, hv.w};
#pragma unroll
            for (int j = 0; j < 4; ++j) {
                float h0 = lo_bf(yw[j]), h1 = hi_bf(yw[j]);
                if (a.resid) {
                    h0 = rbf(lo_bf(hw[j]) + h0);
                    h1 = rbf(hi_bf(hw[j]) + h1);
                }
                ss += h0 * h0;
                ss += h1 * h1;
                ow[j] = pack_bf(h0, h1);
            }
            const float other = __shfl_xor(ss, 1, 64);
            if (m < a.M && otile < n_tiles) {
                *reinterpret_cast<uint4*>(hp) = make_uint4(ow[0], ow[1], ow[2], ow[3]);
                if (p == 0 && a.ss_out) a.ss_out[(size_t)otile * a.ss_ld + m] = ss + other;
            }
        } else {
            if (m >= a.M || otile >= n_tiles) continue;
            if (a.y_tiled)
                *reinterpret_cast<uint4*>(a.y + act_tiled_offset(m, n, a.yMB)) = v;
            else
                *reinterpret_cast<uint4*>(a.y + (size_t)m * a.ldy + n) = v;
        }
    }
    }
    Q3_TL(6);
    Q3_TL_END();
}
```

### swift-qwen3-tts_amd/csrc/kernels/gemm_decode.hip

```cpp
#include "../common.h"
#include "../kernels.h"
#include "row_jobs.h"

namespace q3 {

namespace {

#include "gemm_body.inc"

template <int MB, int EPI, int NW, int CH, bool NORM, bool QUANT, int NP = 1, bool NTW = false, bool TM = false>
__global__ __launch_bounds__(NW * 64) void gemm_skinny_kernel(GemmArgs a) {
    __builtin_amdgcn_s_setprio(3);
    gemm_skinny_body<MB, EPI, NW, CH, NORM, QUANT, NP, NTW, TM>(a, blockIdx.x, blockIdx.y * MB);
}

struct GemmSideArgs {
    GemmArgs g;
    NormRowsArgs n;
    int tiles;
};
template <int MB, int CH, bool QUANT>
__global__ __launch_bounds__(512) void gemm_skinny_side_kernel(GemmSideArgs s) {
    __builtin_amdgcn_s_setprio(3);
    if (int(blockIdx.x) >= s.tiles) {
        __shared__ float side_sh[4];
        __shared__ float side_parts[8];
        if (blockIdx.y == 0) norm_row_job(s.n, int(blockIdx.x) - s.tiles, threadIdx.x, side_sh, side_parts);
        return;
    }
    gemm_skinny_body<MB, 0, 8, CH, true, QUANT, 1, false>(s.g, blockIdx.x, blockIdx.y * MB);
}

template <int MB, int EPI, bool NORM, bool QUANT, bool NTW>
void launch_mb(const GemmArgs& a, const SkinnyGeom& g, hipStream_t st) {
    const dim3 grid(g.gx, g.split);
#define Q3_GEMM(NWv, CHv) \
    hipLaunchKernelGGL((gemm_skinny_kernel<MB, EPI, NWv, CHv, NORM, QUANT, 1, NTW>), grid, dim3(NWv * 64), 0, st, a)
    if constexpr (MB == 4 && !NORM && !NTW) {
        if (g.ch == 0 && g.np == 2) { hipLaunchKernelGGL((gemm_skinny_kernel<4, EPI, 8, 0, false, QUANT, 2, false>), grid, dim3(512), 0, st, a); return; }
        if (g.ch == 0 && g.np == 4) { hipLaunchKernelGGL((gemm_skinny_kernel<4, EPI, 8, 0, false, QUANT, 4, false>), grid, dim3(512), 0, st, a); return; }
    }
    if constexpr (EPI == 2 && MB <= 2) {
        if (g.np > 1) {
            if constexpr (MB == 2 && NORM && !QUANT) {
                if constexpr (NTW) {
                    if (g.tm) { hipLaunchKernelGGL((gemm_skinny_kernel<2, 2, 8, 2, true, false, 3, true, true>), grid, dim3(512), 0, st, a); return; }
                } else {
                    if (g.tm) { hipLaunchKernelGGL((gemm_skinny_kernel<2, 2, 8, 1, true, false, 2, false, true>), grid, dim3(512), 0, st, a); return; }
                }
            }
#define Q3_GEMM_NP(CHv, NPv) hipLaunchKernelGGL((gemm_skinny_kernel<MB, 2, 8, CHv, NORM, QUANT, NPv, NTW>), grid, dim3(512), 0, st, a)
            if (g.ch == 1) { if (g.np == 2) Q3_GEMM_NP(1, 2); else Q3_GEMM_NP(1, 3); }
            else { if (g.np == 2) Q3_GEMM_NP(2, 2); else Q3_GEMM_NP(2, 3); }
#undef Q3_GEMM_NP
            return;
        }
    }
    if (g.nw == 4) {
        Q3_GEMM(4, 1);
    } else {
        switch (g.ch) {
            case 1: Q3_GEMM(8, 1); break;
            case 2: Q3_GEMM(8, 2); break;
            case 3: Q3_GEMM(8, 3); break;
            case 6: Q3_GEMM(8, 6); break;
            default: Q3_GEMM(8, 0); break;
        }
    }
#undef Q3_GEMM
}

template <int EPI, bool NORM, bool QUANT>
void launch_q(const GemmArgs& a, hipStream_t st) {
    const SkinnyGeom g = skinny_geometry(a);
    if (g.ntw) {
        if (g.mbw == 1) launch_mb<1, EPI, NORM, QUANT, true>(a, g, st);
        else launch_mb<2, EPI, NORM, QUANT, true>(a, g, st);
        return;
    }
    switch (g.mbw) {
        case 1: launch_mb<1, EPI, NORM, QUANT, false>(a, g, st); break;
        case 2: launch_mb<2, EPI, NORM, QUANT, false>(a, g, st); break;
        case 3: launch_mb<3, EPI, NORM, QUANT, false>(a, g, st); break;
        case 4: launch_mb<4, EPI, NORM, QUANT, false>(a, g, st); break;
        default: throw Error(3, "gemm_skinny: more than 4 row blocks per workgroup");
    }
}

template <int EPI, bool NORM>
void launch_epi(const GemmArgs& a, hipStream_t st) {
    if (a.Wsb) launch_q<EPI, NORM, true>(a, st);
    else launch_q<EPI, NORM, false>(a, st);
}

}

SkinnyGeom skinny_geometry(const GemmArgs& a) {
    SkinnyGeom g{};
    if (gemm_tall_takes(a)) {
        g.tall = true;
        return g;
    }
    const DebugEnv& env = debug_env();
    const bool norm = a.norm_w != nullptr;
    const int MBt = (a.Mpad + 15) / 16;
    const bool no_split = env.gemm_no_row_split;
    int tiles = a.N / 16;
    if (a.epi == 2) {
        const int t8 = a.N / 8;
        tiles = t8 > 512 ? (t8 + 2) / 3 : (t8 > 256 ? (t8 + 1) / 2 : t8);
    }
    int split = 1;
    if (!no_split) {
        if (MBt % 4 == 0 && tiles * 4 <= 256) split = 4;
        else if (MBt % 2 == 0 && tiles * 2 <= 256) split = 2;
        const int cap = norm ? 2 : 4;
        while (MBt / split > cap || MBt % split != 0) ++split;
    }
    while (MBt / split > 4 || MBt % split != 0) ++split;
    g.split = split;
    g.mbw = MBt / split;
    g.ntw = a.nt_weights && g.mbw <= 2;
    const int KC = a.K / 128;
    g.nw = KC <= 4 ? 4 : 8;
    g.ch = (KC + g.nw - 1) / g.nw;
    g.np = 1;
    const int t = a.epi == 2 ? a.N / 8 : a.N / 16;
    g.gx = t;
    bool shaped = false;
    if (g.mbw == 4 && !norm && !g.ntw && !env.gemm_one_pair && g.nw == 8 && t >= 64) {
        g.np = (((t + 3) / 4) * split <= 128) ? 2 : 4;
        g.ch = 0;
        g.gx = (t + g.np - 1) / g.np;
        shaped = true;
    }
    if (!shaped && a.epi == 2 && g.mbw <= 2) {
        const int np = env.gemm_one_pair ? 1 : (t > 512 ? 3 : (t > 256 ? 2 : 1));
        if (g.nw == 8 && (g.ch == 1 || g.ch == 2) && np > 1) {
            g.np = np;
            g.gx = (t + np - 1) / np;
            shaped = true;
            g.tm = !env.gemm_parent_forms && g.mbw == 2 && norm && !a.Wsb && ((g.ntw && g.ch == 2 && np == 3) || (!g.ntw && g.ch == 1 && np == 2));
        }
    }
    if (!shaped) {
        if (g.nw == 4) g.ch = 1;
        else if (g.ch != 1 && g.ch != 2 && g.ch != 3 && g.ch != 6) g.ch = 0;
    }
    return g;
}

bool gemm_norm_rows_rides(const GemmArgs& a, const NormRowsArgs& n) {
    if (a.epi != 0 || !a.norm_w || a.nt_weights || n.M <= 0 || n.H > 4096) return false;
    if (a.K % 128 != 0 || a.N % 16 != 0) return false;
    const SkinnyGeom g = skinny_geometry(a);
    return !(g.tall || g.nw != 8 || g.np != 1 || (g.ch != 1 && g.ch != 2) || g.mbw < 1 || g.mbw > 2 || g.ntw);
}

bool launch_gemm_skinny_with_norm_rows(const GemmArgs& a, const NormRowsArgs& n, hipStream_t st) {
    if (!gemm_norm_rows_rides(a, n)) return false;
    const SkinnyGeom g = skinny_geometry(a);
    Q3_CHECK(a.ss_in && a.ss_count >= 1 && a.ss_ld >= a.Mpad && a.xMB * 16 >= a.Mpad, 3, "gemm_skinny: norm prologue needs sums of squares");
    const int tiles = g.gx;
    const dim3 grid(tiles + n.M, g.split), block(512);
    const GemmSideArgs s{a, n, tiles};
    const bool q = a.Wsb != nullptr;
#define Q3_SIDE(MBv, CHv)                                                                              \
    do {                                                                                               \
        if (q) hipLaunchKernelGGL((gemm_skinny_side_kernel<MBv, CHv, true>), grid, block, 0, st, s);   \
        else hipLaunchKernelGGL((gemm_skinny_side_kernel<MBv, CHv, false>), grid, block, 0, st, s);    \
    } while (0)
    if (g.mbw == 1) { if (g.ch == 1) Q3_SIDE(1, 1); else Q3_SIDE(1, 2); }
    else { if (g.ch == 1) Q3_SIDE(2, 1); else Q3_SIDE(2, 2); }
#undef Q3_SIDE
    return true;
}

void launch_gemm_skinny(const GemmArgs& a, hipStream_t st) {
    Q3_CHECK(a.K % 128 == 0 && a.N % (a.epi == 2 ? 8 : 16) == 0, 3, "gemm_skinny: K must be a multiple of 128 and N of 16");
    Q3_CHECK(a.Mpad % 16 == 0 && a.M <= a.Mpad && a.Mpad <= 1024, 3, "gemm_skinny: bad M padding");
    Q3_CHECK(a.xMB * 16 >= a.Mpad, 3, "gemm_skinny: x allocation has fewer row blocks than the batch");
    const bool norm = a.norm_w != nullptr;
    if (a.epi == 3) Q3_CHECK(a.yMB * 16 >= a.Mpad, 3, "gemm_skinny: h allocation has fewer row blocks than the batch");
    if (launch_gemm_tall(a, st)) return;
    if (norm) Q3_CHECK(a.ss_in && a.ss_count >= 1 && a.ss_ld >= a.Mpad, 3, "gemm_skinny: norm prologue needs sums of squares");
    switch (a.epi) {
        case 0: norm ? launch_epi<0, true>(a, st) : launch_epi<0, false>(a, st); break;
        case 2: norm ? launch_epi<2, true>(a, st) : launch_epi<2, false>(a, st); break;
        case 3: norm ? launch_epi<3, true>(a, st) : launch_epi<3, false>(a, st); break;
        default: throw Error(3, "gemm_skinny: unknown epilogue");
    }
}

}

#ifdef Q3TTS_GEMM_TIMELINE
extern "C" int q3tts_debug_gemm_timeline(unsigned long long* out) {
    if (hipDeviceSynchronize() != hipSuccess) return 7;
    return hipMemcpyFromSymbol(out, HIP_SYMBOL(q3::g_gemm_tl), sizeof(q3::g_gemm_tl)) == hipSuccess ? 0 : 7;
}
#endif
```

### swift-qwen3-tts_amd/qwen3tts/_lib.py

```python
from __future__ import annotations

import ctypes as C
import os

_HERE = os.path.dirname(os.path.abspath(__file__))
LIB_PATH = os.environ.get("Q3TTS_LIB") or os.path.join(_HERE, "libq3tts_hip.so")

u16p = C.POINTER(C.c_uint16)
i32p = C.POINTER(C.c_int32)
f32p = C.POINTER(C.c_float)
u8p = C.POINTER(C.c_uint8)


class LoadOpts(C.Structure):
    _fields_ = [("device", C.c_int32), ("max_batch", C.c_int32), ("max_frames", C.c_int32),
                ("max_prompt", C.c_int32), ("use_graph", C.c_int32), ("weights_from_broadcast", C.c_int32),
                ("n_streams", C.c_int32), ("codec_overlap_cus", C.c_int32), ("codec_fp32", C.c_int32),
                ("output_sample_rate", C.c_int32), ("speed", C.c_float), ("request_speeds", C.c_int32)]


class LoadOptsEx(C.Structure):
    _fields_ = [("base", LoadOpts), ("pitch", C.c_float)]


class CommId(C.Structure):
    _fields_ = [("bytes", C.c_char * 128)]


class ModelInfo(C.Structure):
    _fields_ = [("tts_model_type", C.c_char * 32), ("sample_rate", C.c_int32),
                ("supports_voice_cloning", C.c_int32), ("has_voice_cloning", C.c_int32),
                ("hidden_size", C.c_int32), ("num_layers", C.c_int32), ("vocab_size", C.c_int32),
                ("text_vocab_size", C.c_int32), ("num_code_groups", C.c_int32),
                ("cp_hidden_size", C.c_int32), ("cp_num_layers", C.c_int32), ("cp_vocab_size", C.c_int32),
                ("codec_eos_token_id", C.c_int32), ("samples_per_frame", C.c_int32), ("max_batch", C.c_int32),
                ("weight_bytes", C.c_int64), ("speaker_embedding_dim", C.c_int32), ("max_samples_per_frame", C.c_int32)]


class Request(C.Structure):
    _fields_ = [("text_ids", i32p), ("n_text_ids", C.c_int32), ("instruct_ids", i32p),
                ("n_instruct_ids", C.c_int32), ("target_token_count", C.c_int32), ("speaker", C.c_char_p),
                ("language", C.c_char_p), ("max_tokens", C.c_int32), ("speed", C.c_float),
                ("ref_audio", f32p), ("n_ref_samples", C.c_int64), ("ref_text_ids", i32p),
                ("n_ref_text_ids", C.c_int32), ("route", C.c_int32)]


ROW_TEMPERATURE, ROW_TOP_K, ROW_TOP_P, ROW_REPETITION_PENALTY, ROW_SEED = 1, 2, 4, 8, 16


class RowSampling(C.Structure):
    _fields_ = [("set", C.c_uint32), ("temperature", C.c_float), ("top_k", C.c_int32), ("top_p", C.c_float),
                ("repetition_penalty", C.c_float), ("seed", C.c_uint64)]


class Sampling(C.Structure):
    _fields_ = [("temperature", C.c_float), ("top_k", C.c_int32), ("top_p", C.c_float),
                ("repetition_penalty", C.c_float), ("seed", C.c_uint64), ("force_frames", C.c_int32), ("audio_chunk_frames", C.c_int32),
                ("audio_window_frames", C.c_int32), ("audio_lookahead_frames", C.c_int32), ("row_base", C.c_uint32),
                ("per_request", C.POINTER(RowSampling)), ("audio_stream_reference", C.c_int32)]


class GenInfo(C.Structure):
    _fields_ = [("prompt_token_count", C.c_int32), ("generation_token_count", C.c_int32),
                ("prefill_time", C.c_double), ("generate_time", C.c_double), ("tokens_per_second", C.c_double),
                ("peak_memory_usage", C.c_double)]


class Event(C.Structure):
    _fields_ = [("kind", C.c_int), ("request_index", C.c_int32), ("token", C.c_int32),
                ("info", C.POINTER(GenInfo)), ("pcm", f32p), ("n_samples", C.c_int64), ("sample_offset", C.c_int64)]


EVENT_CB = C.CFUNCTYPE(None, C.c_void_p, C.POINTER(Event))


class Result(C.Structure):
    _fields_ = [("status", C.c_int), ("pcm", f32p), ("n_samples", C.c_int64), ("codes", i32p),
                ("n_frames", C.c_int32), ("info", GenInfo)]


class Timing(C.Structure):
    _fields_ = [("prefill_ms", C.c_double), ("decode_ms", C.c_double), ("codec_ms", C.c_double),
                ("frame_steps", C.c_int32), ("rows", C.c_int32), ("kv_bytes_read", C.c_int64),
                ("frontend_ms", C.c_double), ("first_audio_ms", C.c_double), ("launches_per_frame_step", C.c_int32)]


class VoiceInfo(C.Structure):
    _fields_ = [("ref_frames", C.c_int32), ("ref_text_tokens", C.c_int32), ("n_ref_samples", C.c_int64),
                ("device_bytes", C.c_int64)]


class SessionOpts(C.Structure):
    _fields_ = [("slots", C.c_int32), ("max_pending", C.c_int32), ("max_ref_frames", C.c_int32)]


class SessionStats(C.Structure):
    _fields_ = [("submitted", C.c_int64), ("pending", C.c_int64), ("running", C.c_int64), ("completed", C.c_int64),
                ("cancelled", C.c_int64), ("frame_steps", C.c_int64), ("admissions", C.c_int64)]


class SessionTextStats(C.Structure):
    _fields_ = [("open", C.c_int64), ("starved", C.c_int64), ("appended_tokens", C.c_int64), ("starve_events", C.c_int64)]


ERR_CANCELLED, ERR_BUSY = 8, 9


class AttnDebug(C.Structure):
    _fields_ = [("n_heads", C.c_int32), ("n_kv", C.c_int32), ("B", C.c_int32), ("eps", C.c_float), ("scale", C.c_float),
                ("max_pages", C.c_int32), ("fixed_len", C.c_int32), ("identity_pages", C.c_int32), ("chunk", C.c_int32),
                ("chunk_r_base", C.c_int32), ("nt_kv", C.c_int32), ("n_pos", C.c_int32), ("n_pages", C.c_int32),
                ("qkv", u16p), ("qn_w", u16p), ("kn_w", u16p), ("rope_cos", u16p), ("rope_sin", u16p),
                ("kv_len", i32p), ("active", u8p), ("block_table", i32p), ("chunk_n_prompt", i32p),
                ("kpool", u16p), ("vpool", u16p), ("out", u16p)]


class GemmDebug(C.Structure):
    _fields_ = [("mode", C.c_int32), ("geometry_only", C.c_int32), ("M", C.c_int32), ("K", C.c_int32), ("N", C.c_int32),
                ("xMB", C.c_int32), ("yMB", C.c_int32), ("ss_ld", C.c_int32), ("y_cols", C.c_int32),
                ("epi", C.c_int32), ("act_silu", C.c_int32), ("resid", C.c_int32), ("nt_weights", C.c_int32), ("y_tiled", C.c_int32),
                ("norm", C.c_int32), ("quant", C.c_int32), ("has_bias", C.c_int32), ("ss_count", C.c_int32), ("norm_dim", C.c_int32),
                ("norm_eps", C.c_float),
                ("rider_M", C.c_int32), ("rider_H", C.c_int32), ("rider_MB", C.c_int32), ("rider_ss_count", C.c_int32),
                ("rider_eps", C.c_float),
                ("rode", C.c_int32), ("tall", C.c_int32), ("tall_shape", C.c_int32),
                ("split", C.c_int32), ("mbw", C.c_int32), ("nw", C.c_int32), ("ch", C.c_int32), ("np", C.c_int32), ("gx", C.c_int32),
                ("ntw", C.c_int32), ("tm", C.c_int32),
                ("x", u16p), ("W", C.c_void_p), ("scales", u16p), ("biases", u16p), ("W_up", C.c_void_p), ("scales_up", u16p),
                ("biases_up", u16p), ("bias", u16p), ("norm_w", u16p), ("ss_in", f32p), ("rider_h", u16p), ("rider_w", u16p),
                ("rider_ss_in", f32p),
                ("y", u16p), ("ss_out", f32p), ("rider_out", u16p), ("rider_ss_out", f32p)]


class ConvDebug(C.Structure):
    _fields_ = [("kind", C.c_int32), ("geometry_only", C.c_int32), ("split", C.c_int32),
                ("B", C.c_int32), ("Tmax", C.c_int32), ("ppf", C.c_int32), ("hist", C.c_int32), ("margin", C.c_int32),
                ("Cin", C.c_int32), ("N", C.c_int32), ("K", C.c_int32), ("dil", C.c_int32),
                ("ldx", C.c_int32), ("ldo", C.c_int32), ("ldr", C.c_int32), ("ldx2", C.c_int32),
                ("act", C.c_int32), ("pre_act", C.c_int32), ("shift", C.c_int32), ("reflect", C.c_int32), ("post_C", C.c_int32),
                ("x_f32", C.c_int32), ("res_is_out", C.c_int32),
                ("family", C.c_int32), ("BN", C.c_int32), ("pro", C.c_int32), ("pw_depth", C.c_int32), ("KT", C.c_int32),
                ("X32", C.c_int32), ("CT2", C.c_int32), ("PT", C.c_int32), ("wdb", C.c_int32),
                ("grid_x", C.c_int32), ("grid_y", C.c_int32), ("grid_z", C.c_int32), ("lds_bytes", C.c_int64),
                ("frames", i32p), ("x", C.c_void_p), ("x2", f32p), ("w", f32p), ("w2", f32p), ("bias", f32p), ("bias2", f32p),
                ("scale", f32p), ("snake_alpha", f32p), ("snake_beta", f32p), ("act2_alpha", f32p), ("act2_beta", f32p),
                ("post_alpha", f32p), ("post_beta", f32p), ("res", C.c_void_p),
                ("out", C.c_void_p), ("out2", C.c_void_p), ("pcm", f32p), ("nonfinite", i32p)]


class RowopDebug(C.Structure):
    _fields_ = [("op", C.c_int32), ("check_only", C.c_int32), ("p", C.c_int32 * 16), ("f", C.c_float * 4),
                ("in", C.c_void_p * 8), ("in_bytes", C.c_int64 * 8), ("io", C.c_void_p * 4), ("io_bytes", C.c_int64 * 4)]


ROWOPS = ("rvq_gather", "rmsnorm_f32", "dwconv_ln", "silu_mul_f32", "attn_full_f32", "roll_history", "roll_history_rows",
          "history_state_rows", "stream_take_chunk", "enc_init_conv", "layernorm_f32", "rope_qk_f32", "attn_causal_f32", "rvq_encode",
          "log_mel", "time_stats", "scale_res", "asp_concat", "asp_pool", "mask_tail", "copy2d_f32")


def rowop(handle, op, p, f, ins, ios, check_only=False):
    a = RowopDebug(op=ROWOPS.index(op), check_only=1 if check_only else 0)
    for i, v in enumerate(p):
        a.p[i] = int(v)
    for i, v in enumerate(f):
        a.f[i] = float(v)
    inp = getattr(a, "in")
    for i, v in enumerate(ins):
        if v is not None:
            assert v.flags["C_CONTIGUOUS"]
            inp[i], a.in_bytes[i] = v.ctypes.data, v.nbytes
    for i, v in enumerate(ios):
        if v is not None:
            assert v.flags["C_CONTIGUOUS"] and v.flags["WRITEABLE"]
            a.io[i], a.io_bytes[i] = v.ctypes.data, v.nbytes
    return lib().q3tts_debug_rowop(handle, C.byref(a))


class LmSamplingParams(C.Structure):
    _fields_ = [("temperature", C.c_float), ("top_k", C.c_int32), ("top_p", C.c_float), ("rep_penalty", C.c_float),
                ("seed", C.c_uint64), ("row0", C.c_uint32), ("mask_eos", C.c_int32)]


class LmAdmitDesc(C.Structure):
    _fields_ = [("slot", C.c_int32), ("n_trailing", C.c_int32), ("max_frames", C.c_int32), ("row_key", C.c_uint32),
                ("text_open", C.c_int32), ("pad_", C.c_int32), ("sp", LmSamplingParams)]


class LmTextDesc(C.Structure):
    _fields_ = [("slot", C.c_int32), ("src_row", C.c_int32), ("n_new", C.c_int32), ("close", C.c_int32),
                ("max_frames", C.c_int32), ("pad_", C.c_int32)]


class LmopDebug(C.Structure):
    _fields_ = [("op", C.c_int32), ("check_only", C.c_int32), ("p", C.c_int32 * 32),
                ("in", C.c_void_p * 14), ("in_bytes", C.c_int64 * 14), ("io", C.c_void_p * 18), ("io_bytes", C.c_int64 * 18)]


LMOPS = ("sampler", "sampler_frame_end", "frame_end", "gather_rows", "tile_rows", "untile_rows", "add_rows", "compose_rows",
         "ref_embed_rows", "f32_to_bf16", "ss_to_table", "copy_rows", "prefill_load", "prefill_chunk_load", "advance_len",
         "advance_len_chunk", "admit_rows", "text_append_rows", "cancel_rows")


def lmop(handle, op, p, ins, ios, check_only=False):
    a = LmopDebug(op=LMOPS.index(op), check_only=1 if check_only else 0)
    for i, v in p.items():
        a.p[i] = int(v)
    inp = getattr(a, "in")
    for i, v in ins.items():
        if v is not None:
            assert v.flags["C_CONTIGUOUS"]
            inp[i], a.in_bytes[i] = v.ctypes.data, v.nbytes
    for i, v in ios.items():
        if v is not None:
            assert v.flags["C_CONTIGUOUS"] and v.flags["WRITEABLE"]
            a.io[i], a.io_bytes[i] = v.ctypes.data, v.nbytes
    return lib().q3tts_debug_lmop(handle, C.byref(a))


_lib = None


def lib() -> C.CDLL:
    global _lib
    if _lib is not None:
        return _lib
    if not os.path.exists(LIB_PATH):
        raise RuntimeError(f"{LIB_PATH} is missing: build the HIP engine first "
                           "(make -C swift-qwen3-tts_amd); there is no CPU fallback")
    L = C.CDLL(LIB_PATH)
    vp = C.c_void_p
    L.q3tts_default_load_opts.argtypes = [C.POINTER(LoadOpts)]
    L.q3tts_default_sampling.argtypes = [C.POINTER(Sampling)]
    L.q3tts_model_load.argtypes = [C.c_char_p, C.POINTER(LoadOpts), C.POINTER(vp)]
    L.q3tts_model_free.argtypes = [vp]
    L.q3tts_model_free.restype = None
    L.q3tts_last_error.argtypes = [vp]
    L.q3tts_last_error.restype = C.c_char_p
    L.q3tts_model_arena.argtypes = [vp, C.POINTER(vp), C.POINTER(C.c_size_t)]
    L.q3tts_model_get_info.argtypes = [vp, C.POINTER(ModelInfo)]
    L.q3tts_comm_get_unique_id.argtypes = [C.POINTER(CommId)]
    L.q3tts_model_broadcast.argtypes = [vp, C.POINTER(CommId), C.c_int32, C.c_int32, C.c_int32]
    L.q3tts_model_arena_checksum.argtypes = [vp, C.POINTER(C.c_uint64)]
    L.q3tts_model_num_speakers.argtypes = [vp]
    L.q3tts_model_speaker_name.argtypes = [vp, C.c_int32]
    L.q3tts_model_speaker_name.restype = C.c_char_p
    L.q3tts_generate.argtypes = [vp, C.POINTER(Request), C.c_int32, C.POINTER(Sampling), EVENT_CB, vp,
                                 C.POINTER(Result)]
    L.q3tts_generate_queued.argtypes = [vp, C.POINTER(Request), C.c_int32, C.c_int32, C.POINTER(Sampling), EVENT_CB, vp,
                                        C.POINTER(Result)]
    L.q3tts_voice_create.argtypes = [vp, f32p, C.c_int64, i32p, C.c_int32, C.POINTER(vp)]
    if hasattr(L, "q3tts_resample"):
        L.q3tts_voice_create_rate.argtypes = [vp, f32p, C.c_int64, C.c_int32, i32p, C.c_int32, C.POINTER(vp)]
        L.q3tts_resample.argtypes = [vp, f32p, C.c_int64, C.c_int32, C.c_int32, C.c_int32, f32p, C.c_int64, C.POINTER(C.c_int64)]
    if hasattr(L, "q3tts_time_stretch"):
        L.q3tts_model_get_speed.argtypes = [vp, C.POINTER(C.c_float), C.POINTER(C.c_int32), C.POINTER(C.c_int32)]
        L.q3tts_time_stretch.argtypes = [vp, f32p, C.c_int64, C.c_float, C.c_int32, f32p, C.c_int64, C.POINTER(C.c_int64)]
    L.q3tts_voice_free.argtypes = [vp, vp]
    L.q3tts_voice_free.restype = None
    L.q3tts_voice_get_info.argtypes = [vp, C.POINTER(VoiceInfo)]
    L.q3tts_generate_voices.argtypes = [vp, C.POINTER(Request), C.POINTER(vp), C.c_int32, C.POINTER(Sampling), EVENT_CB, vp,
                                        C.POINTER(Result)]
    L.q3tts_generate_queued_voices.argtypes = [vp, C.POINTER(Request), C.POINTER(vp), C.c_int32, C.c_int32, C.POINTER(Sampling),
                                               EVENT_CB, vp, C.POINTER(Result)]
    if hasattr(L, "q3tts_session_open"):
        L.q3tts_session_open.argtypes = [vp, C.POINTER(SessionOpts), C.POINTER(Sampling), EVENT_CB, vp, C.POINTER(vp)]
        L.q3tts_session_submit.argtypes = [vp, C.POINTER(Request), vp, C.POINTER(RowSampling), C.POINTER(C.c_int64)]
        L.q3tts_session_cancel.argtypes = [vp, C.c_int64]
        L.q3tts_session_wait.argtypes = [vp, C.c_int64, C.c_int32, C.POINTER(Result), i32p]
        L.q3tts_session_get_stats.argtypes = [vp, C.POINTER(SessionStats)]
        L.q3tts_session_close.argtypes = [vp, C.c_int32]
    if hasattr(L, "q3tts_session_submit_open"):
        L.q3tts_session_submit_open.argtypes = [vp, C.POINTER(Request), C.POINTER(RowSampling), C.POINTER(C.c_int64)]
        L.q3tts_session_append_text.argtypes = [vp, C.c_int64, i32p, C.c_int32, C.c_int32]
        L.q3tts_session_get_text_stats.argtypes = [vp, C.POINTER(SessionTextStats)]
        L.q3tts_debug_text_resume.argtypes = [vp, C.c_int32, C.c_int32, u16p, i32p, u16p, u16p, f32p, i32p]
    L.q3tts_generate_begin.argtypes = [vp, C.POINTER(Request), C.c_int32, C.POINTER(Sampling), EVENT_CB, vp, C.c_int32, C.POINTER(vp)]
    L.q3tts_generate_end.argtypes = [vp, vp, C.POINTER(Result)]
    L.q3tts_pcm_to_int16.argtypes = [f32p, C.c_int64, C.POINTER(C.c_int16)]
    L.q3tts_pcm_to_int16.restype = None
    L.q3tts_write_wav.argtypes = [C.c_char_p, f32p, C.c_int64, C.c_int32]
    L.q3tts_result_free.argtypes = [C.POINTER(Result), C.c_int32]
    L.q3tts_result_free.restype = None
    L.q3tts_codec_decode.argtypes = [vp, i32p, i32p, C.c_int32, C.c_int32, f32p, C.POINTER(C.c_int64)]
    L.q3tts_codec_decode_streamed.argtypes = [vp, i32p, i32p, C.c_int32, C.c_int32, C.c_int32, C.c_int32, C.c_int32, f32p]
    if hasattr(L, "q3tts_codec_decode_streamed_prefixed"):
        L.q3tts_codec_decode_streamed_prefixed.argtypes = [vp, i32p, i32p, i32p, C.c_int32, C.c_int32, C.c_int32, C.c_int32, C.c_int32,
                                                           f32p]
    if hasattr(L, "q3tts_request_speed_info"):
        L.q3tts_request_speed_info.argtypes = [vp, C.c_float, C.POINTER(C.c_float), i32p, i32p, i32p]
        L.q3tts_debug_stretch_rows.argtypes = [vp, f32p, i32p, i32p, C.c_int32, C.c_int64, f32p, C.c_int64]
    if hasattr(L, "q3tts_pitch_shift"):
        L.q3tts_default_load_opts_ex.argtypes = [C.POINTER(LoadOptsEx)]
        L.q3tts_default_load_opts_ex.restype = None
        L.q3tts_model_load_ex.argtypes = [C.c_char_p, C.POINTER(LoadOptsEx), C.POINTER(vp)]
        L.q3tts_model_get_pitch.argtypes = [vp, C.POINTER(C.c_float), i32p, i32p, i32p]
        L.q3tts_pitch_shift.argtypes = [vp, f32p, C.c_int64, C.c_float, f32p, C.c_int64, C.POINTER(C.c_int64)]
        L.q3tts_debug_resample_ratio.argtypes = [vp, f32p, i32p, C.c_int32, C.c_int64, C.c_int64, C.c_int64, C.c_int32, C.c_int32, C.c_int32,
                                                 f32p, C.c_int64]
    if hasattr(L, "q3tts_debug_prefix_states"):
        L.q3tts_debug_prefix_states.argtypes = [vp, i32p, C.POINTER(C.c_int64), C.POINTER(C.c_int64)]
    if hasattr(L, "q3tts_debug_codec_stream_slots"):
        L.q3tts_debug_codec_stream_slots.argtypes = [vp, i32p, i32p, C.c_int32, C.c_int32, C.c_int32, C.c_int32, C.c_int32, C.c_int32,
                                                     C.c_int32, f32p]
    L.q3tts_debug_set_codec_scratch.argtypes = [C.c_uint64]
    L.q3tts_debug_set_codec_scratch.restype = None
    L.q3tts_debug_reload_env.argtypes = []
    L.q3tts_debug_reload_env.restype = None
    L.q3tts_last_timing.argtypes = [vp, C.POINTER(Timing)]
    L.q3tts_codec_encode.argtypes = [vp, f32p, C.c_int64, i32p, C.c_int32, i32p]
    L.q3tts_codec_encoded_frames.argtypes = [vp, C.c_int64]
    L.q3tts_speaker_embedding.argtypes = [vp, f32p, C.c_int64, C.c_int32, f32p, C.c_int32]
    L.q3tts_debug_frontend_stage.argtypes = [vp, f32p, C.c_int64, C.c_char_p, f32p, C.c_int64, i32p, i32p]
    L.q3tts_tokenizer_load.argtypes = [C.c_char_p, C.POINTER(vp)]
    L.q3tts_tokenizer_free.argtypes = [vp]
    L.q3tts_tokenizer_free.restype = None
    L.q3tts_tokenizer_encode.argtypes = [vp, C.c_char_p, i32p, C.c_int32, i32p]
    L.q3tts_debug_prepare_inputs.argtypes = [vp, C.POINTER(Request), u16p, C.c_int32, i32p, u16p, C.c_int32,
                                             i32p, u16p]
    L.q3tts_debug_generate_forced.argtypes = [vp, C.POINTER(Request), C.c_int32, C.POINTER(Sampling), i32p,
                                              C.c_int32, u16p, u16p, i32p]
    L.q3tts_debug_sample.argtypes = [vp, u16p, C.c_int32, C.c_int32, C.POINTER(Sampling), u8p, C.c_int32,
                                     C.c_int32, C.c_int32, C.c_uint32, C.c_uint32, i32p]
    L.q3tts_debug_linear.argtypes = [vp, u16p, u16p, u16p, C.c_int32, C.c_int32, C.c_int32, u16p]
    L.q3tts_debug_attention.argtypes = [vp, C.POINTER(AttnDebug)]
    if hasattr(L, "q3tts_debug_gemm"):
        L.q3tts_debug_gemm.argtypes = [vp, C.POINTER(GemmDebug)]
    if hasattr(L, "q3tts_debug_conv"):
        L.q3tts_debug_conv.argtypes = [vp, C.POINTER(ConvDebug)]
    if hasattr(L, "q3tts_debug_rowop"):
        L.q3tts_debug_rowop.argtypes = [vp, C.POINTER(RowopDebug)]
    if hasattr(L, "q3tts_debug_lmop"):
        L.q3tts_debug_lmop.argtypes = [vp, C.POINTER(LmopDebug)]
    if hasattr(L, "q3tts_debug_build_decode_codes"):
        L.q3tts_debug_build_decode_codes.argtypes = [vp, i32p, i32p, i32p, i32p, C.c_int32, C.c_int32, C.c_int32, C.c_int32, i32p]
    L.q3tts_debug_codec_stage.argtypes = [vp, i32p, C.c_int32, C.c_char_p, f32p, C.c_int64, i32p, i32p]
    _lib = L
    return L


GEOM_FIELDS = ("rode", "tall", "tall_shape", "split", "mbw", "nw", "ch", "np", "gx", "ntw", "tm")


def gemm_geometry(**kw) -> dict:
    a = GemmDebug(geometry_only=1, **kw)
    st = lib().q3tts_debug_gemm(None, C.byref(a))
    if st != 0:
        raise ValueError("q3tts_debug_gemm refused the arguments (status %d): %r" % (st, kw))
    return {f: int(getattr(a, f)) for f in GEOM_FIELDS}


CONV_GEOM_FIELDS = ("family", "BN", "pro", "pw_depth", "KT", "X32", "CT2", "PT", "wdb", "grid_x", "grid_y", "grid_z", "lds_bytes")
CONV_OPERANDS = ("x2", "bias", "bias2", "scale", "snake", "act2", "post", "res", "out", "out2", "w2", "pcm", "nonfinite")


def conv_geometry(frames=None, **kw) -> dict:
    ops = {k: kw.pop(k, False) for k in CONV_OPERANDS}
    a = ConvDebug(geometry_only=1, **kw)
    one = (C.c_float * 4)()
    fp = C.cast(one, f32p)
    a.w = fp
    for name in ("x2", "bias", "bias2", "scale", "w2", "pcm"):
        if ops[name]:
            setattr(a, name, fp)
    for name in ("snake", "act2", "post"):
        if ops[name]:
            setattr(a, name + "_alpha", fp)
            setattr(a, name + "_beta", fp)
    for name in ("res", "out", "out2"):
        if ops[name]:
            setattr(a, name, C.cast(one, C.c_void_p))
    if ops["nonfinite"]:
        a.nonfinite = C.cast(one, i32p)
    fr = None
    if frames is not None:
        fr = (C.c_int32 * len(frames))(*frames)
        a.frames = C.cast(fr, i32p)
    st = lib().q3tts_debug_conv(None, C.byref(a))
    if st != 0:
        raise ValueError("q3tts_debug_conv refused the arguments (status %d): %r" % (st, kw))
    return {f: int(getattr(a, f)) for f in CONV_GEOM_FIELDS}


def reload_debug_env() -> None:
    lib().q3tts_debug_reload_env()
```

Baseline: 10670.

## Add lean prologue/epilogue variant for decode skinny GEMM kernels

```diff
diff --git a/include/q3tts.h b/include/q3tts.h
--- a/include/q3tts.h
+++ b/include/q3tts.h
@@ -334,6 +334,7 @@
     int32_t tall_shape;
     int32_t split, mbw, nw, ch, np, gx, ntw;
     int32_t tm;
+    int32_t lean;
     const uint16_t* x;
     const void* W;
     const uint16_t* scales;
diff --git a/swift-qwen3-tts_amd/csrc/debug_env.cc b/swift-qwen3-tts_amd/csrc/debug_env.cc
--- a/swift-qwen3-tts_amd/csrc/debug_env.cc
+++ b/swift-qwen3-tts_amd/csrc/debug_env.cc
@@ -21,6 +21,7 @@
     d->gemm_no_row_split = flag("Q3TTS_GEMM_NO_ROW_SPLIT");
     d->gemm_one_pair = flag("Q3TTS_GEMM_ONE_PAIR");
     d->gemm_parent_forms = number("Q3TTS_GEMM_PARENT_FORMS", 0) != 0;
+    d->gemm_parent_prologue_epilogue = number("Q3TTS_GEMM_PARENT_PROLOGUE_EPILOGUE", 0) != 0;
     d->no_tall_gemm = flag("Q3TTS_NO_TALL_GEMM");
     d->tall_shape = number("Q3TTS_TALL_SHAPE", 0);
     d->chunk_qsplit = number("Q3TTS_CHUNK_QSPLIT", 0);
diff --git a/swift-qwen3-tts_amd/csrc/engine_debug.cc b/swift-qwen3-tts_amd/csrc/engine_debug.cc
--- a/swift-qwen3-tts_amd/csrc/engine_debug.cc
+++ b/swift-qwen3-tts_amd/csrc/engine_debug.cc
@@ -308,7 +308,7 @@
 void Engine::debug_gemm_check(q3tts_gemm_debug& d, GemmArgs& ga, NormRowsArgs& na) {
     static const uint16_t dummy16 = 0;
     static const uint32_t dummy32 = 0;
-    d.rode = d.tall = d.tall_shape = d.split = d.mbw = d.nw = d.ch = d.np = d.gx = d.ntw = d.tm = 0;
+    d.rode = d.tall = d.tall_shape = d.split = d.mbw = d.nw = d.ch = d.np = d.gx = d.ntw = d.tm = d.lean = 0;
     Q3_CHECK(d.mode == 0 || d.mode == 1, 3, "debug_gemm: unknown mode");
     const bool rider = d.mode == 1 || d.rider_M > 0;
     if (rider) {
@@ -355,7 +355,7 @@
         d.tall_shape = gemm_tall_shape(ga);
     } else {
         Q3_CHECK(g.mbw >= 1 && g.mbw <= 4, 3, "debug_gemm: more than 4 row blocks per workgroup");
-        d.split = g.split; d.mbw = g.mbw; d.nw = g.nw; d.ch = g.ch; d.np = g.np; d.gx = g.gx; d.ntw = g.ntw ? 1 : 0; d.tm = g.tm ? 1 : 0;
+        d.split = g.split; d.mbw = g.mbw; d.nw = g.nw; d.ch = g.ch; d.np = g.np; d.gx = g.gx; d.ntw = g.ntw ? 1 : 0; d.tm = g.tm ? 1 : 0; d.lean = g.lean ? 1 : 0;
     }
     if (rider) d.rode = gemm_norm_rows_rides(ga, na) ? 1 : 0;
 }
diff --git a/swift-qwen3-tts_amd/csrc/kernels.h b/swift-qwen3-tts_amd/csrc/kernels.h
--- a/swift-qwen3-tts_amd/csrc/kernels.h
+++ b/swift-qwen3-tts_amd/csrc/kernels.h
@@ -9,6 +9,7 @@
     bool gemm_no_row_split;
     bool gemm_one_pair;
     bool gemm_parent_forms;
+    bool gemm_parent_prologue_epilogue;
     bool no_tall_gemm;
     int tall_shape;
     int chunk_qsplit;
@@ -66,6 +67,7 @@
     int gx;
     bool ntw;
     bool tm;
+    bool lean;
 };
 SkinnyGeom skinny_geometry(const GemmArgs& a);
 bool launch_gemm_skinny_with_norm_rows(const GemmArgs& a, const NormRowsArgs& n, hipStream_t st);
diff --git a/swift-qwen3-tts_amd/csrc/kernels/attn_body.inc b/swift-qwen3-tts_amd/csrc/kernels/attn_body.inc
--- a/swift-qwen3-tts_amd/csrc/kernels/attn_body.inc
+++ b/swift-qwen3-tts_amd/csrc/kernels/attn_body.inc
@@ -10,6 +10,35 @@
     o0 = rbf(rbf(y0 * bf2f(cosr[lane])) + rbf(-y1 * bf2f(sinr[lane])));
     o1 = rbf(rbf(y1 * bf2f(cosr[lane + 64])) + rbf(y0 * bf2f(sinr[lane + 64])));
 }
+
+#ifdef Q3TTS_GEMM_TIMELINE
+__device__ unsigned long long g_attn_tl[2][4][8];
+#define Q3_ATL_BEGIN()                                               \
+    constexpr bool kAtl = REP == 2 && NTH == 256 && !NTKV;           \
+    unsigned long long atl_[8] = {0, 0, 0, 0, 0, 0, 0, 0};           \
+    Q3_ATL(0)
+#define Q3_ATL(k)                                  \
+    do {                                           \
+        if constexpr (kAtl) {                      \
+            __builtin_amdgcn_sched_barrier(0);     \
+            atl_[k] = wall_clock64();              \
+            __builtin_amdgcn_sched_barrier(0);     \
+        }                                          \
+    } while (0)
+#define Q3_ATL_END()                                                                                                 \
+    do {                                                                                                             \
+        if constexpr (kAtl) {                                                                                        \
+            const bool atl_last = blockIdx.x == gridDim.x - 1 && blockIdx.y == gridDim.y - 1;                        \
+            if ((atl_last || (blockIdx.x == 0 && blockIdx.y == 0)) && (threadIdx.x & 63) == 0) {                     \
+                _Pragma("unroll") for (int k = 0; k < 8; ++k) g_attn_tl[atl_last ? 1 : 0][threadIdx.x >> 6][k] = atl_[k]; \
+            }                                                                                                        \
+        }                                                                                                            \
+    } while (0)
+#else
+#define Q3_ATL_BEGIN() ((void)0)
+#define Q3_ATL(k) ((void)0)
+#define Q3_ATL_END() ((void)0)
+#endif
 
 template <int REP, int NTH, bool NTKV = false>
 __device__ __forceinline__ void attn_decode_body(const AttnArgs& a, const int kvh, const int b) {
@@ -23,6 +52,7 @@
     __shared__ float acc_s[NG][REP][D];
 
     const int tid = threadIdx.x, lane = tid & 63, wave = tid >> 6;
+    Q3_ATL_BEGIN();
     const int len = a.fixed_len >= 0 ? a.fixed_len : a.kv_len[b];
     const bool append = a.active ? (a.active[b] != 0) : true;
     const uint16_t* row = a.qkv + (size_t)b * a.ld;
@@ -100,7 +130,9 @@
             }
         }
     }
+    Q3_ATL(1);
     __syncthreads();
+    Q3_ATL(2);
 
     float q[REP][8];
 #pragma unroll
@@ -170,6 +202,7 @@
         step(kf, vf);
     }
 
+    Q3_ATL(3);
 #pragma unroll
     for (int h = 0; h < REP; ++h) {
         if (c == 0) {
@@ -180,6 +213,7 @@
         for (int j = 0; j < 8; ++j) acc_s[g][h][8 * c + j] = acc[h][j];
     }
     __syncthreads();
+    Q3_ATL(4);
 
     uint16_t* out_s = reinterpret_cast<uint16_t*>(&q_s[0][0]);
     for (int o = tid; o < REP * D; o += NTH) {
@@ -196,9 +230,13 @@
         }
         out_s[o] = f2bf(num / den);
     }
+    Q3_ATL(5);
     __syncthreads();
+    Q3_ATL(6);
     for (int p = tid; p < REP * D / 8; p += NTH) {
         const int col = (kvh * REP) * D + 8 * p;
         *reinterpret_cast<uint4*>(a.out + act_tiled_offset(b, col, a.outMB)) = *reinterpret_cast<const uint4*>(out_s + 8 * p);
     }
+    Q3_ATL(7);
+    Q3_ATL_END();
 }
diff --git a/swift-qwen3-tts_amd/csrc/kernels/attn_decode.hip b/swift-qwen3-tts_amd/csrc/kernels/attn_decode.hip
--- a/swift-qwen3-tts_amd/csrc/kernels/attn_decode.hip
+++ b/swift-qwen3-tts_amd/csrc/kernels/attn_decode.hip
@@ -211,3 +211,10 @@
 }
 
 }
+
+#ifdef Q3TTS_GEMM_TIMELINE
+extern "C" int q3tts_debug_attn_timeline(unsigned long long* out) {
+    if (hipDeviceSynchronize() != hipSuccess) return 7;
+    return hipMemcpyFromSymbol(out, HIP_SYMBOL(q3::g_attn_tl), sizeof(q3::g_attn_tl)) == hipSuccess ? 0 : 7;
+}
+#endif
diff --git a/swift-qwen3-tts_amd/csrc/kernels/gemm_body.inc b/swift-qwen3-tts_amd/csrc/kernels/gemm_body.inc
--- a/swift-qwen3-tts_amd/csrc/kernels/gemm_body.inc
+++ b/swift-qwen3-tts_amd/csrc/kernels/gemm_body.inc
@@ -1,10 +1,16 @@
 #ifdef Q3TTS_GEMM_TIMELINE
-__device__ unsigned long long g_gemm_tl[4][2][8][8];
+__device__ unsigned long long g_gemm_tl[9][2][8][9];
 #define Q3_TL_BEGIN()                                                                                                       \
+    constexpr bool kTlPred = !QUANT && !NTW && NW == 8;                                                                     \
     constexpr int kTlForm = (EPI == 2 && MB == 2 && NW == 8 && CH == 2 && NP == 3 && NTW) ? (TM ? 1 : 0)                    \
-                            : ((EPI == 3 && MB == 1 && NW == 8 && CH == 6 && !NORM && NTW) ? 2                              \
-                               : ((EPI == 0 && MB == 2 && NW == 8 && CH == 2 && NORM && NP == 1 && NTW) ? 3 : -1));         \
-    unsigned long long tl_[8] = {0, 0, 0, 0, 0, 0, 0, 0};                                                                   \
+                            : (EPI == 3 && MB == 1 && NW == 8 && CH == 6 && !NORM && NTW) ? 2                               \
+                            : (EPI == 0 && MB == 2 && NW == 8 && CH == 2 && NORM && NP == 1 && NTW) ? 3                     \
+                            : (kTlPred && EPI == 0 && MB == 2 && CH == 1 && NORM && NP == 1) ? 4                            \
+                            : (kTlPred && EPI == 3 && MB == 1 && CH == 2 && !NORM && NP == 1) ? 5                           \
+                            : (kTlPred && EPI == 2 && MB == 2 && CH == 1 && NORM && NP == 2 && TM) ? 6                      \
+                            : (kTlPred && EPI == 3 && MB == 1 && CH == 3 && !NORM && NP == 1) ? 7                           \
+                            : (kTlPred && EPI == 0 && MB == 1 && CH == 1 && NORM && NP == 1) ? 8 : -1;                      \
+    unsigned long long tl_[9] = {0, 0, 0, 0, 0, 0, 0, 0, 0};                                                                \
     Q3_TL(0)
 #define Q3_TL(k)                                   \
     do {                                           \
@@ -19,7 +25,7 @@
         if constexpr (kTlForm >= 0) {                                                                                       \
             const bool tl_last = blockIdx.x == gridDim.x - 1 && blockIdx.y == gridDim.y - 1;                                \
             if ((tl_last || (blockIdx.x == 0 && blockIdx.y == 0)) && lane == 0) {                                           \
-                _Pragma("unroll") for (int k = 0; k < 8; ++k) g_gemm_tl[kTlForm][tl_last ? 1 : 0][wave][k] = tl_[k];        \
+                _Pragma("unroll") for (int k = 0; k < 9; ++k) g_gemm_tl[kTlForm][tl_last ? 1 : 0][wave][k] = tl_[k];        \
             }                                                                                                               \
         }                                                                                                                   \
     } while (0)
@@ -38,6 +44,16 @@
 
 __device__ __forceinline__ float silu_f(float v) { return v / (1.0f + __expf(-v)); }
 
+template <int N>
+__device__ __forceinline__ uint32_t dpp_row_shl(uint32_t v) {
+    return (uint32_t)__builtin_amdgcn_update_dpp((int)v, (int)v, 0x100 + N, 0xF, 0xF, false);
+}
+__device__ __forceinline__ uint4 gather_piece(uint16_t yb) {
+    const uint32_t y = yb;
+    const uint32_t w = y | (dpp_row_shl<1>(y) << 16);
+    return make_uint4(w, dpp_row_shl<2>(w), dpp_row_shl<4>(w), dpp_row_shl<6>(w));
+}
+
 __device__ __forceinline__ uint4 norm8(const uint4& hx, const uint4& wx, float rstd) {
     const uint32_t hw[4] = {hx.x, hx.y, hx.z, hx.w}, ww[4] = {wx.x, wx.y, wx.z, wx.w};
     uint32_t o[4];
@@ -64,8 +80,9 @@
     }
 }
 
-template <int MB, int EPI, int NW, int CH, bool NORM, bool QUANT, int NP = 1, bool NTW = false, bool TM = false>
+template <int MB, int EPI, int NW, int CH, bool NORM, bool QUANT, int NP = 1, bool NTW = false, bool TM = false, bool LEAN = false>
 __device__ __forceinline__ void gemm_skinny_body(const GemmArgs& a, const int tile, const int mb0) {
+    static_assert(!LEAN || (MB <= 2 && !QUANT && CH > 0), "the lean prologue / epilogue is a decode form");
     constexpr int NT = NP;
     constexpr int NR = 1;
     constexpr int NB = TM ? NT : 1;
@@ -73,7 +90,7 @@
     static_assert(!TM || (EPI == 2 && NORM && !QUANT && CH > 0 && NP > 1), "tile-major order is a gate/up form");
     const int n_tiles = (EPI == 2) ? (a.N >> 3) : (a.N >> 4);
     __shared__ float red[NB][NW][NR][MB][4][64];
-    __shared__ __attribute__((aligned(16))) uint16_t ys[NB][MB][16][16];
+    __shared__ __attribute__((aligned(16))) uint16_t ys[LEAN ? 1 : NB][LEAN ? 1 : MB][16][16];
     __shared__ float rstd_s[NORM ? 16 * MB : 1];
     __shared__ float ssp_s[NORM ? 8 : 1][NORM ? 16 * MB : 1];
 
@@ -93,7 +110,25 @@
 
     constexpr int kSsIter = NORM ? (16 * MB * 8 + NW * 64 - 1) / (NW * 64) : 1;
     float sst[kSsIter][16];
-    if constexpr (NORM) {
+    const int wave_u = LEAN ? __builtin_amdgcn_readfirstlane(threadIdx.x >> 6) : 0;
+    constexpr int kSsU = (LEAN && CH * NW < 16) ? CH * NW : 16;
+    static_assert(!LEAN || !NORM || (kSsIter == 1 && 2 * MB <= NW), "one slot per thread of the first 2 * MB waves");
+    if constexpr (NORM && LEAN) {
+        if (wave_u < 2 * MB) {
+            const int rows = 16 * MB;
+            const int row = threadIdx.x % rows, part = threadIdx.x / rows;
+            const float* sp = a.ss_in + 16 * mb0 + row;
+            sst[0][0] = sp[(size_t)(part < a.ss_count ? part : 0) * a.ss_ld];
+            if (a.ss_count > 8) {
+#pragma unroll
+                for (int u = 1; u < kSsU; ++u) {
+                    const int j = part + 8 * u;
+                    sst[0][u] = sp[(size_t)(j < a.ss_count ? j : 0) * a.ss_ld];
+                }
+            }
+        }
+        __builtin_amdgcn_sched_barrier(0);
+    } else if constexpr (NORM) {
         const int rows = 16 * MB;
 #pragma unroll
         for (int it = 0; it < kSsIter; ++it) {
@@ -179,7 +214,19 @@
     }
     __builtin_amdgcn_sched_barrier(0);
     uint4 hv_pre = make_uint4(0, 0, 0, 0);
-    if constexpr (EPI == 3 && NT == 1) {
+    constexpr int kTrips = (256 * MB + NW * 64 - 1) / (NW * 64);
+    uint4 hv_lean[LEAN ? kTrips : 1];
+    if constexpr (EPI == 3 && NT == 1 && LEAN) {
+#pragma unroll
+        for (int tr = 0; tr < kTrips; ++tr) {
+            hv_lean[tr] = make_uint4(0, 0, 0, 0);
+            const int o = threadIdx.x + tr * NW * 64;
+            if (a.resid && wave_u + tr * NW < 4 * MB && (lane & 7) == 0) {
+                const int mb = o >> 8, b = (o >> 4) & 15, p = (o >> 3) & 1;
+                hv_lean[tr] = *reinterpret_cast<const uint4*>(a.y + act_tiled_offset(16 * (mb0 + mb) + b, tile * 16 + 8 * p, a.yMB));
+            }
+        }
+    } else if constexpr (EPI == 3 && NT == 1) {
         if (a.resid && threadIdx.x < 32 * MB) {
             const int o = threadIdx.x, mb = o >> 5, b = (o >> 1) & 15, p = o & 1;
             hv_pre = *reinterpret_cast<const uint4*>(a.y + act_tiled_offset(16 * (mb0 + mb) + b, tile * 16 + 8 * p, a.yMB));
@@ -189,6 +236,17 @@
     float rstd[MB];
     if constexpr (NORM) {
         const int rows = 16 * MB;
+        if constexpr (LEAN) {
+            if (wave_u < 2 * MB) {
+                const int row = threadIdx.x % rows, part = threadIdx.x / rows;
+                float s = 0.f;
+#pragma unroll
+                for (int u = 0; u < kSsU; ++u)
+                    if (part + 8 * u < a.ss_count) s += sst[0][u];
+                for (int j = part + 8 * kSsU; j < a.ss_count; j += 8) s += a.ss_in[(size_t)j * a.ss_ld + 16 * mb0 + row];
+                ssp_s[part][row] = s;
+            }
+        } else {
 #pragma unroll
         for (int it = 0; it < kSsIter; ++it) {
             const int idx = threadIdx.x + it * NW * 64;
@@ -202,6 +260,8 @@
                 ssp_s[part][row] = s;
             }
         }
+        }
+        Q3_TL(8);
         __syncthreads();
         if (threadIdx.x < rows) {
             float s = 0.f;
@@ -345,6 +405,82 @@
     if (pr == NT / NR - 1) Q3_TL(4);
     const int otile = tile * (NT / NR) + pr;
 
+    if constexpr (LEAN && EPI == 2) {
+        static_assert(128 * MB <= NW * 64, "one pass");
+        if (wave_u < 2 * MB) {
+            const int o = threadIdx.x;
+            const int mb = o >> 7, rem = o & 127;
+            const int b = rem >> 3, f = rem & 7;
+            const int lg = (f >> 2) * 16 + b, lu = (2 + (f >> 2)) * 16 + b, q = f & 3;
+            float g = 0.f, u = 0.f;
+#pragma unroll
+            for (int w = 0; w < NW; ++w) {
+                g += red[rb][w][0][mb][q][lg];
+                u += red[rb][w][0][mb][q][lu];
+            }
+            const uint4 v = gather_piece(f2bf(rbf(silu_f(rbf(g))) * rbf(u)));
+            if (pr == 0) Q3_TL(7);
+            if (pr == NT / NR - 1) Q3_TL(5);
+            const int m = 16 * (mb0 + mb) + b;
+            if (f == 0 && m < a.M && otile < n_tiles) *reinterpret_cast<uint4*>(a.y + act_tiled_offset(m, otile * 8, a.yMB)) = v;
+        }
+    } else if constexpr (LEAN) {
+#pragma unroll
+        for (int tr = 0; tr < kTrips; ++tr) {
+            if (wave_u + tr * NW >= 4 * MB) continue;
+            const int o = threadIdx.x + tr * NW * 64;
+            const int mb = o >> 8, rem = o & 255;
+            const int b = rem >> 4, f = rem & 15;
+            const int src_lane = (f >> 2) * 16 + b, q = f & 3;
+            float sum = 0.f;
+#pragma unroll
+            for (int w = 0; w < NW; ++w) sum += red[rb][w][0][mb][q][src_lane];
+            float y = sum;
+            if (a.bias && otile < n_tiles) y += bf2f(a.bias[otile * 16 + f]);
+            uint16_t yb = f2bf(y);
+            if (EPI == 0 && a.act_silu) yb = f2bf(silu_f(bf2f(yb)));
+            const uint4 v = gather_piece(yb);
+            if (pr == 0) Q3_TL(7);
+            if (pr == NT / NR - 1) Q3_TL(5);
+            const int p = f >> 3;
+            const bool storer = (f & 7) == 0;
+            const int m = 16 * (mb0 + mb) + b;
+            const int n = otile * 16 + 8 * p;
+            if constexpr (EPI == 3) {
+                uint16_t* hp = a.y + act_tiled_offset(m, n, a.yMB);
+                float ss = 0.f;
+                const uint32_t yw[4] = {v.x, v.y, v.z, v.w};
+                uint32_t ow[4];
+                uint4 hv = hv_lean[tr];
+                if constexpr (NT > 1) {
+                    if (a.resid && storer && m < a.M && otile < n_tiles) hv = *reinterpret_cast<const uint4*>(hp);
+                }
+                const uint32_t hw[4] = {hv.x, hv.y, hv.z, hv.w};
+#pragma unroll
+                for (int j = 0; j < 4; ++j) {
+                    float h0 = lo_bf(yw[j]), h1 = hi_bf(yw[j]);
+                    if (a.resid) {
+                        h0 = rbf(lo_bf(hw[j]) + h0);
+                        h1 = rbf(hi_bf(hw[j]) + h1);
+                    }
+                    ss += h0 * h0;
+                    ss += h1 * h1;
+                    ow[j] = pack_bf(h0, h1);
+                }
+                const float other = XorPartner::x8(ss);
+                if (storer && m < a.M && otile < n_tiles) {
+                    *reinterpret_cast<uint4*>(hp) = make_uint4(ow[0], ow[1], ow[2], ow[3]);
+                    if (p == 0 && a.ss_out) a.ss_out[(size_t)otile * a.ss_ld + m] = ss + other;
+                }
+            } else {
+                if (!storer || m >= a.M || otile >= n_tiles) continue;
+                if (a.y_tiled)
+                    *reinterpret_cast<uint4*>(a.y + act_tiled_offset(m, n, a.yMB)) = v;
+                else
+                    *reinterpret_cast<uint4*>(a.y + (size_t)m * a.ldy + n) = v;
+            }
+        }
+    } else {
     if constexpr (EPI == 2) {
         for (int o = threadIdx.x; o < 128 * MB; o += NW * 64) {
             const int mb = o >> 7, rem = o & 127;
@@ -425,6 +561,7 @@
         }
     }
     }
+    }
     Q3_TL(6);
     Q3_TL_END();
 }
diff --git a/swift-qwen3-tts_amd/csrc/kernels/gemm_decode.hip b/swift-qwen3-tts_amd/csrc/kernels/gemm_decode.hip
--- a/swift-qwen3-tts_amd/csrc/kernels/gemm_decode.hip
+++ b/swift-qwen3-tts_amd/csrc/kernels/gemm_decode.hip
@@ -12,6 +12,19 @@
 __global__ __launch_bounds__(NW * 64) void gemm_skinny_kernel(GemmArgs a) {
     __builtin_amdgcn_s_setprio(3);
     gemm_skinny_body<MB, EPI, NW, CH, NORM, QUANT, NP, NTW, TM>(a, blockIdx.x, blockIdx.y * MB);
+}
+
+template <int MB, int EPI, int NW, int CH, bool NORM, int NP>
+constexpr int kLeanWavesPerSimd = (MB == 2 && NW == 8 && NP == 1 && (CH == 1 || (CH == 2 && (EPI == 0 || !NORM)))) ? 4 : 1;
+template <int MB, int EPI, int NW, int CH, bool NORM, int NP = 1, bool NTW = false, bool TM = false>
+__global__ __launch_bounds__(NW * 64, (kLeanWavesPerSimd<MB, EPI, NW, CH, NORM, NP>)) void gemm_skinny_lean_kernel(GemmArgs a) {
+    __builtin_amdgcn_s_setprio(3);
+    gemm_skinny_body<MB, EPI, NW, CH, NORM, false, NP, NTW, TM, true>(a, blockIdx.x, blockIdx.y * MB);
+}
+template <bool LEAN, int MB, int EPI, int NW, int CH, bool NORM, bool QUANT, int NP, bool NTW, bool TM = false>
+constexpr auto skinny_kernel() {
+    if constexpr (LEAN) return &gemm_skinny_lean_kernel<MB, EPI, NW, CH, NORM, NP, NTW, TM>;
+    else return &gemm_skinny_kernel<MB, EPI, NW, CH, NORM, QUANT, NP, NTW, TM>;
 }
 
 struct GemmSideArgs {
@@ -30,12 +43,23 @@
     }
     gemm_skinny_body<MB, 0, 8, CH, true, QUANT, 1, false>(s.g, blockIdx.x, blockIdx.y * MB);
 }
-
-template <int MB, int EPI, bool NORM, bool QUANT, bool NTW>
+template <int MB, int CH>
+__global__ __launch_bounds__(512, (kLeanWavesPerSimd<MB, 0, 8, CH, true, 1>)) void gemm_skinny_side_lean_kernel(GemmSideArgs s) {
+    __builtin_amdgcn_s_setprio(3);
+    if (int(blockIdx.x) >= s.tiles) {
+        __shared__ float side_sh[4];
+        __shared__ float side_parts[8];
+        if (blockIdx.y == 0) norm_row_job(s.n, int(blockIdx.x) - s.tiles, threadIdx.x, side_sh, side_parts);
+        return;
+    }
+    gemm_skinny_body<MB, 0, 8, CH, true, false, 1, false, false, true>(s.g, blockIdx.x, blockIdx.y * MB);
+}
+
+template <int MB, int EPI, bool NORM, bool QUANT, bool NTW, bool LEAN = false>
 void launch_mb(const GemmArgs& a, const SkinnyGeom& g, hipStream_t st) {
     const dim3 grid(g.gx, g.split);
 #define Q3_GEMM(NWv, CHv) \
-    hipLaunchKernelGGL((gemm_skinny_kernel<MB, EPI, NWv, CHv, NORM, QUANT, 1, NTW>), grid, dim3(NWv * 64), 0, st, a)
+    hipLaunchKernelGGL((skinny_kernel<LEAN, MB, EPI, NWv, CHv, NORM, QUANT, 1, NTW>()), grid, dim3(NWv * 64), 0, st, a)
     if constexpr (MB == 4 && !NORM && !NTW) {
         if (g.ch == 0 && g.np == 2) { hipLaunchKernelGGL((gemm_skinny_kernel<4, EPI, 8, 0, false, QUANT, 2, false>), grid, dim3(512), 0, st, a); return; }
         if (g.ch == 0 && g.np == 4) { hipLaunchKernelGGL((gemm_skinny_kernel<4, EPI, 8, 0, false, QUANT, 4, false>), grid, dim3(512), 0, st, a); return; }
@@ -44,12 +68,12 @@
         if (g.np > 1) {
             if constexpr (MB == 2 && NORM && !QUANT) {
                 if constexpr (NTW) {
-                    if (g.tm) { hipLaunchKernelGGL((gemm_skinny_kernel<2, 2, 8, 2, true, false, 3, true, true>), grid, dim3(512), 0, st, a); return; }
+                    if (g.tm) { hipLaunchKernelGGL((skinny_kernel<LEAN, 2, 2, 8, 2, true, false, 3, true, true>()), grid, dim3(512), 0, st, a); return; }
                 } else {
-                    if (g.tm) { hipLaunchKernelGGL((gemm_skinny_kernel<2, 2, 8, 1, true, false, 2, false, true>), grid, dim3(512), 0, st, a); return; }
+                    if (g.tm) { hipLaunchKernelGGL((skinny_kernel<LEAN, 2, 2, 8, 1, true, false, 2, false, true>()), grid, dim3(512), 0, st, a); return; }
                 }
             }
-#define Q3_GEMM_NP(CHv, NPv) hipLaunchKernelGGL((gemm_skinny_kernel<MB, 2, 8, CHv, NORM, QUANT, NPv, NTW>), grid, dim3(512), 0, st, a)
+#define Q3_GEMM_NP(CHv, NPv) hipLaunchKernelGGL((skinny_kernel<LEAN, MB, 2, 8, CHv, NORM, QUANT, NPv, NTW>()), grid, dim3(512), 0, st, a)
             if (g.ch == 1) { if (g.np == 2) Q3_GEMM_NP(1, 2); else Q3_GEMM_NP(1, 3); }
             else { if (g.np == 2) Q3_GEMM_NP(2, 2); else Q3_GEMM_NP(2, 3); }
 #undef Q3_GEMM_NP
@@ -64,7 +88,10 @@
             case 2: Q3_GEMM(8, 2); break;
             case 3: Q3_GEMM(8, 3); break;
             case 6: Q3_GEMM(8, 6); break;
-            default: Q3_GEMM(8, 0); break;
+            default:
+                if constexpr (LEAN) throw Error(3, "gemm_skinny: the streamed form has no lean variant");
+                else Q3_GEMM(8, 0);
+                break;
         }
     }
 #undef Q3_GEMM
@@ -73,6 +100,18 @@
 template <int EPI, bool NORM, bool QUANT>
 void launch_q(const GemmArgs& a, hipStream_t st) {
     const SkinnyGeom g = skinny_geometry(a);
+    if constexpr (!QUANT) {
+        if (g.lean) {
+            if (g.ntw) {
+                if (g.mbw == 1) launch_mb<1, EPI, NORM, false, true, true>(a, g, st);
+                else launch_mb<2, EPI, NORM, false, true, true>(a, g, st);
+            } else {
+                if (g.mbw == 1) launch_mb<1, EPI, NORM, false, false, true>(a, g, st);
+                else launch_mb<2, EPI, NORM, false, false, true>(a, g, st);
+            }
+            return;
+        }
+    }
     if (g.ntw) {
         if (g.mbw == 1) launch_mb<1, EPI, NORM, QUANT, true>(a, g, st);
         else launch_mb<2, EPI, NORM, QUANT, true>(a, g, st);
@@ -147,6 +186,7 @@
         if (g.nw == 4) g.ch = 1;
         else if (g.ch != 1 && g.ch != 2 && g.ch != 3 && g.ch != 6) g.ch = 0;
     }
+    g.lean = !env.gemm_parent_prologue_epilogue && a.Mpad <= 32 && g.mbw <= 2 && !a.Wsb && g.ch != 0;
     return g;
 }
 
@@ -165,10 +205,11 @@
     const dim3 grid(tiles + n.M, g.split), block(512);
     const GemmSideArgs s{a, n, tiles};
     const bool q = a.Wsb != nullptr;
-#define Q3_SIDE(MBv, CHv)                                                                              \
-    do {                                                                                               \
-        if (q) hipLaunchKernelGGL((gemm_skinny_side_kernel<MBv, CHv, true>), grid, block, 0, st, s);   \
-        else hipLaunchKernelGGL((gemm_skinny_side_kernel<MBv, CHv, false>), grid, block, 0, st, s);    \
+#define Q3_SIDE(MBv, CHv)                                                                                          \
+    do {                                                                                                           \
+        if (q) hipLaunchKernelGGL((gemm_skinny_side_kernel<MBv, CHv, true>), grid, block, 0, st, s);               \
+        else if (g.lean) hipLaunchKernelGGL((gemm_skinny_side_lean_kernel<MBv, CHv>), grid, block, 0, st, s); \
+        else hipLaunchKernelGGL((gemm_skinny_side_kernel<MBv, CHv, false>), grid, block, 0, st, s);                \
     } while (0)
     if (g.mbw == 1) { if (g.ch == 1) Q3_SIDE(1, 1); else Q3_SIDE(1, 2); }
     else { if (g.ch == 1) Q3_SIDE(2, 1); else Q3_SIDE(2, 2); }
diff --git a/swift-qwen3-tts_amd/qwen3tts/_lib.py b/swift-qwen3-tts_amd/qwen3tts/_lib.py
--- a/swift-qwen3-tts_amd/qwen3tts/_lib.py
+++ b/swift-qwen3-tts_amd/qwen3tts/_lib.py
@@ -125,7 +125,7 @@
                 ("rider_eps", C.c_float),
                 ("rode", C.c_int32), ("tall", C.c_int32), ("tall_shape", C.c_int32),
                 ("split", C.c_int32), ("mbw", C.c_int32), ("nw", C.c_int32), ("ch", C.c_int32), ("np", C.c_int32), ("gx", C.c_int32),
-                ("ntw", C.c_int32), ("tm", C.c_int32),
+                ("ntw", C.c_int32), ("tm", C.c_int32), ("lean", C.c_int32),
                 ("x", u16p), ("W", C.c_void_p), ("scales", u16p), ("biases", u16p), ("W_up", C.c_void_p), ("scales_up", u16p),
                 ("biases_up", u16p), ("bias", u16p), ("norm_w", u16p), ("ss_in", f32p), ("rider_h", u16p), ("rider_w", u16p),
                 ("rider_ss_in", f32p),
@@ -338,7 +338,7 @@
     return L
 
 
-GEOM_FIELDS = ("rode", "tall", "tall_shape", "split", "mbw", "nw", "ch", "np", "gx", "ntw", "tm")
+GEOM_FIELDS = ("rode", "tall", "tall_shape", "split", "mbw", "nw", "ch", "np", "gx", "ntw", "tm", "lean")
 
 
 def gemm_geometry(**kw) -> dict:
```

After: 10590. No clear change (-0.7%).
